# tfzhou/ContrastiveSeg

Measured on AMD Instinct MI355X. Metric: images/sec contrastive train step, HRNet-W48 1024x512 bs8, higher is better.
Workload: dtype fp32 in/out, f16x3 split MFMA (fp32 accumulate); 1 GPU; cfg2: BASELINE.json configs[1]: HRNet-W48 + contrast_ce_loss, synthetic Cityscapes 3x512x1024x19, tau=0.1, max_samples=1024, with_embed=True, SGD(0.01,0.9,5; model=hrnet_w48_contrast, loss=contrast_ce_loss, global_batch=8, per_gpu_batch=8, arithmetic=f16x3 on the matrix cores for the 3x3 / 1x1 convolutions, rest fp32, parallelism=dp1, step_graph=eager (auto: per-GPU batch above 1, the GPU is the limit)

## Files before the change

### contrastiveseg_amd/_hip.py

```python
import ctypes
import os

import torch

_PKG = os.path.dirname(os.path.abspath(__file__))
LIB_PATH = os.path.join(_PKG, "libcseg_hip.so")

_c_int = ctypes.c_int
_c_float = ctypes.c_float
_ptr = ctypes.c_void_p


class ContrastDesc(ctypes.Structure):
    _fields_ = [("mode", _c_int), ("N", _c_int), ("M", _c_int), ("D", _c_int),
                ("anchors", _ptr), ("a_lab", _ptr), ("contrast", _ptr), ("c_lab", _ptr),
                ("segment_queue", _ptr), ("pixel_queue", _ptr),
                ("bank_classes", _c_int), ("bank_size", _c_int),
                ("temperature", _c_float), ("base_temperature", _c_float)]


class ConvGroupMember(ctypes.Structure):
    _fields_ = [("x", _ptr), ("wp", _ptr), ("bias", _ptr), ("addend", _ptr), ("y", _ptr), ("stats", _ptr), ("amax_x", _ptr),
                ("amax_w", _ptr), ("B", _c_int), ("Cin", _c_int), ("Cout", _c_int), ("H", _c_int), ("W", _c_int),
                ("reserved", _c_int * 3)]


class BnGroupMember(ctypes.Structure):
    _fields_ = [("x", _ptr), ("residual", _ptr), ("y", _ptr), ("stats", _ptr), ("mean_invstd", _ptr), ("weight", _ptr), ("bias", _ptr),
                ("running_mean", _ptr), ("running_var", _ptr), ("num_batches_tracked", _ptr), ("amax_out", _ptr), ("dy", _ptr),
                ("out", _ptr), ("g_masked", _ptr), ("d_weight", _ptr), ("d_bias", _ptr), ("dx", _ptr), ("ws", _ptr),
                ("B", _c_int), ("C", _c_int), ("HW", _c_int), ("T", ctypes.c_long), ("eps", _c_float), ("momentum", _c_float)]


class WrwGroupMember(ctypes.Structure):
    _fields_ = [("x", _ptr), ("dy", _ptr), ("amax_x", _ptr), ("amax_dy", _ptr), ("ws", _ptr), ("dw", _ptr), ("B", _c_int), ("Cin", _c_int),
                ("Cout", _c_int), ("H", _c_int), ("W", _c_int), ("reserved", _c_int * 3)]


GROUP_MAX = 8
GROUP_SCHED_INTS = 320
NT_GROUP = 0x203


SIGNATURES = {
    "cseg_abi_version": (_c_int, []),
    "cseg_last_error": (ctypes.c_char_p, []),
    "cseg_classify_partition": (_c_int, [_ptr, _ptr, _ptr] + [_c_int] * 7 + [_ptr] * 7 + [_ptr]),
    "cseg_classify_partition_prezeroed": (_c_int, [_ptr, _ptr, _ptr] + [_c_int] * 7 + [_ptr] * 7 + [_ptr]),
    "cseg_gather_anchors": (_c_int, [_ptr, _c_int, _c_int, _c_int, _ptr, _ptr, _c_int, _ptr, _ptr, _ptr]),
    "cseg_scatter_anchor_grad": (_c_int, [_ptr, _c_int, _ptr, _c_int, _c_int, _c_int, _c_float, _ptr, _ptr]),
    "cseg_contrast_ws_bytes": (ctypes.c_size_t, [_c_int, _c_int]),
    "cseg_contrast_fwd": (_c_int, [ctypes.POINTER(ContrastDesc), _ptr, _ptr, _ptr, _ptr, _ptr]),
    "cseg_contrast_fused_ws_bytes": (ctypes.c_size_t, [_c_int, _c_int]),
    "cseg_contrast_fused_counter_offset": (ctypes.c_size_t, [_c_int, _c_int]),
    "cseg_contrast_fwd_fused": (_c_int, [ctypes.POINTER(ContrastDesc), _ptr, _ptr, _ptr, _ptr, _ptr, _ptr]),
    "cseg_contrast_bwd_parts": (_c_int, [_c_int, _c_int, _c_int]),
    "cseg_contrast_bwd": (_c_int, [ctypes.POINTER(ContrastDesc), _ptr, _ptr, _ptr, _ptr, _ptr]),
    "cseg_sampling_ws_ints": (ctypes.c_size_t, [_c_int] * 3),
    "cseg_sample_anchors": (_c_int, [_ptr, _ptr, _ptr] + [_c_int] * 5 + [_ptr] * 7 + [_ptr]),
    "cseg_mt_draw": (_c_int, [_ptr, _ptr, _ptr, _c_int, _ptr]),
    "cseg_gather_anchors_dn": (_c_int, [_ptr, _c_int, _c_int, _c_int, _ptr, _ptr, _ptr, _c_int, _ptr, _ptr, _ptr]),
    "cseg_contrast_fwd_dn": (_c_int, [_ptr, _ptr, _ptr, _c_int, _c_int, _c_float, _c_float, _ptr, _ptr, _ptr, _ptr, _ptr]),
    "cseg_contrast_bwd_parts_cap": (_c_int, [_c_int, _c_int]),
    "cseg_contrast_bwd_dn": (_c_int, [_ptr, _ptr, _ptr, _c_int, _c_int, _c_float, _ptr, _ptr, _ptr, _ptr, _ptr]),
    "cseg_scatter_anchor_grad_dn": (_c_int, [_ptr, _ptr, _ptr, _c_int, _c_int, _c_int, _c_int, _c_float, _ptr, _ptr]),
    "cseg_upcat_fwd": (_c_int, [_ptr, _ptr, _ptr, _ptr, _c_int, _c_int, _ptr, _ptr]),
    "cseg_upcat_fwd_amax": (_c_int, [_ptr, _ptr, _ptr, _ptr, _c_int, _c_int, _ptr, _ptr, _ptr]),
    "cseg_upcat_bwd": (_c_int, [_ptr, _ptr, _ptr, _ptr, _c_int, _c_int, _ptr, _ptr]),
    "cseg_fuse_sum_fwd": (_c_int, [_ptr, _c_int, _ptr, _ptr, _ptr, _c_int] + [_c_int] * 5 + [_ptr, _ptr]),
    "cseg_affine_channels": (_c_int, [_ptr, _ptr, _ptr, _c_int, _c_int, ctypes.c_long, _ptr, _ptr, _ptr]),
    "cseg_fuse_sum_fwd_amax": (_c_int, [_ptr, _c_int, _ptr, _ptr, _ptr, _c_int] + [_c_int] * 5 + [_ptr, _ptr, _ptr]),
    "cseg_fuse_sum_bwd": (_c_int, [_ptr, _ptr, _ptr, _ptr, _c_int] + [_c_int] * 4 + [_ptr, _ptr, _ptr]),
    "cseg_upsample_ce_blocks": (_c_int, [_c_int, _c_int, _c_int]),
    "cseg_upsample_ce_fwd": (_c_int, [_ptr, _ptr, _ptr, _c_int] + [_c_int] * 6 + [_ptr, _ptr, _ptr, _ptr, _ptr]),
    "cseg_upsample_ce_bwd": (_c_int, [_ptr, _ptr, _ptr, _c_int] + [_c_int] * 6 + [_ptr, _ptr, _ptr, _ptr, _ptr]),
    "cseg_queue_count": (_c_int, [_ptr, _c_int, _c_int, _c_int, _c_int, _c_int, _ptr, _ptr]),
    "cseg_queue_class_sums": (_c_int, [_ptr, _ptr] + [_c_int] * 7 + [_ptr, _ptr]),
    "cseg_queue_write_segments": (_c_int, [_ptr, _ptr, _ptr, _ptr, _ptr, _c_int, _c_int, _c_int, _ptr, _c_int, _ptr]),
    "cseg_queue_write_pixels": (_c_int, [_ptr, _c_int, _c_int, _c_int, _ptr, _ptr, _ptr, _ptr, _c_int, _ptr, _c_int,
                                         _ptr]),
    "cseg_conv3x3_packed_floats": (ctypes.c_size_t, [_c_int, _c_int]),
    "cseg_conv3x3_pack_weights": (_c_int, [_ptr, _c_int, _c_int, _c_int, _ptr, _ptr]),
    "cseg_conv3x3_fwd": (_c_int, [_ptr, _ptr, _c_int, _c_int, _c_int, _c_int, _c_int, _ptr, _ptr]),
    "cseg_conv3x3_wrw_ws_floats": (ctypes.c_size_t, [_c_int] * 5),
    "cseg_conv3x3_wrw": (_c_int, [_ptr, _ptr, _c_int, _c_int, _c_int, _c_int, _c_int, _ptr, _ptr, _ptr]),
    "cseg_conv3x3_sb_packed_bytes": (ctypes.c_size_t, [_c_int, _c_int]),
    "cseg_conv3x3_sb_pack_weights": (_c_int, [_ptr, _c_int, _c_int, _c_int, _ptr, _ptr]),
    "cseg_conv3x3_sb_fwd": (_c_int, [_ptr, _ptr, _ptr, _c_int, _c_int, _c_int, _c_int, _c_int, _ptr, _ptr]),
    "cseg_conv3x3_sb_pack_weights_nt": (_c_int, [_ptr, _c_int, _c_int, _c_int, _c_int, _ptr, _ptr]),
    "cseg_conv3x3_sb_fwd_nt": (_c_int, [_ptr, _ptr, _ptr, _c_int, _c_int, _c_int, _c_int, _c_int, _c_int, _ptr, _ptr]),
    "cseg_conv3x3_sb_wrw_ws_floats": (ctypes.c_size_t, [_c_int] * 5),
    "cseg_conv3x3_sb_wrw": (_c_int, [_ptr, _ptr, _c_int, _c_int, _c_int, _c_int, _c_int, _ptr, _ptr, _ptr]),
    "cseg_conv1x1_sb_packed_bytes": (ctypes.c_size_t, [_c_int, _c_int]),
    "cseg_conv1x1_sb_pack_weights": (_c_int, [_ptr, _c_int, _c_int, _c_int, _ptr, _ptr]),
    "cseg_conv1x1_sb_fwd": (_c_int, [_ptr, _ptr, _ptr, _c_int, _c_int, _c_int, _c_int, _ptr, _ptr]),
    "cseg_conv1x1_sb_wrw_ws_floats": (ctypes.c_size_t, [_c_int] * 4),
    "cseg_conv1x1_sb_wrw": (_c_int, [_ptr, _ptr, _c_int, _c_int, _c_int, _c_int, _ptr, _ptr, _ptr]),
    "cseg_amax_f32": (_c_int, [_ptr, ctypes.c_long, _ptr, _ptr]),
    "cseg_conv3x3_split_packed_bytes": (ctypes.c_size_t, [_c_int, _c_int, _c_int]),
    "cseg_conv3x3_split_pack": (_c_int, [_ptr, _c_int, _c_int, _c_int, _c_int, _c_int, _ptr, _ptr, _ptr]),
    "cseg_conv3x3_split_fwd": (_c_int, [_ptr, _ptr, _ptr] + [_c_int] * 7 + [_ptr, _ptr, _ptr, _ptr]),
    "cseg_conv3x3_split_wrw": (_c_int, [_ptr, _ptr] + [_c_int] * 6 + [_ptr, _ptr, _ptr, _ptr, _ptr]),
    "cseg_conv3x3_split_fwd_add": (_c_int, [_ptr, _ptr, _ptr, _ptr] + [_c_int] * 7 + [_ptr, _ptr, _ptr, _ptr]),
    "cseg_conv3x3_split_group_fwd": (_c_int, [_ptr, _c_int, _c_int, _ptr, _ptr]),
    "cseg_conv3x3_split_group_wrw": (_c_int, [_ptr, _c_int, _c_int, _ptr]),
    "cseg_bn_group_tiles_finalize": (_c_int, [_ptr, _c_int, _ptr]),
    "cseg_bn_group_apply": (_c_int, [_ptr, _c_int, _c_int, _ptr]),
    "cseg_bn_group_bwd": (_c_int, [_ptr, _c_int, _c_int, _c_int, _ptr]),
    "cseg_bn_group_tiles_moments": (_c_int, [_ptr, _c_int, _ptr, _ptr]),
    "cseg_bn_group_finalize": (_c_int, [_ptr, _c_int, _ptr, _ptr]),
    "cseg_bn_group_bwd_reduce": (_c_int, [_ptr, _c_int, _c_int, _ptr, _ptr]),
    "cseg_bn_group_bwd_apply": (_c_int, [_ptr, _c_int, _c_int, _ptr, _ptr]),
    "cseg_conv3x3_split_dil_fwd": (_c_int, [_ptr, _ptr, _ptr, _ptr] + [_c_int] * 7 + [_ptr, _ptr, _ptr, _ptr, _ptr]),
    "cseg_conv3x3_split_dilany_plan": (_c_int, [_c_int, _c_int, ctypes.POINTER(_c_int), ctypes.POINTER(ctypes.c_long)]),
    "cseg_conv3x3_split_dilany_packed_bytes": (ctypes.c_size_t, [_c_int] * 2),
    "cseg_conv3x3_split_dilany_pack": (_c_int, [_ptr, _c_int, _c_int, _c_int, _ptr, _ptr, _ptr]),
    "cseg_conv3x3_split_dilany_fwd": (_c_int, [_ptr, _ptr, _ptr, _ptr] + [_c_int] * 6 + [_ptr, _ptr, _ptr, _ptr, _ptr]),
    "cseg_conv3x3_split_dilany_wrw_ws_floats": (ctypes.c_size_t, [_c_int] * 6),
    "cseg_conv3x3_split_dilany_wrw": (_c_int, [_ptr, _ptr] + [_c_int] * 6 + [_ptr, _ptr, _ptr, _ptr, _ptr]),
    "cseg_conv3x3_s2_split_packed_bytes": (ctypes.c_size_t, [_c_int] * 2),
    "cseg_conv3x3_s2_split_plan": (_c_int, [_c_int] * 4 + [_ptr, _ptr]),
    "cseg_conv3x3_s2_split_pack": (_c_int, [_ptr] + [_c_int] * 4 + [_ptr, _ptr, _ptr]),
    "cseg_conv3x3_s2_split_fwd": (_c_int, [_ptr, _ptr] + [_c_int] * 6 + [_ptr, _ptr, _ptr, _ptr]),
    "cseg_conv3x3_s2_split_bwd": (_c_int, [_ptr, _ptr] + [_c_int] * 6 + [_ptr, _ptr, _ptr, _ptr]),
    "cseg_conv3x3_s2_rgb_fwd": (_c_int, [_ptr, _ptr] + [_c_int] * 4 + [_ptr, _ptr]),
    "cseg_conv3x3_s2_rgb_wrw_ws_floats": (ctypes.c_size_t, [_c_int] * 4),
    "cseg_conv3x3_s2_rgb_wrw": (_c_int, [_ptr, _ptr] + [_c_int] * 4 + [_ptr, _ptr, _ptr]),
    "cseg_cls1x1_fwd": (_c_int, [_ptr, _ptr, _ptr] + [_c_int] * 4 + [ctypes.c_long, _ptr, _ptr]),
    "cseg_cls1x1_bwd": (_c_int, [_ptr, _ptr] + [_c_int] * 4 + [ctypes.c_long, _ptr, _ptr]),
    "cseg_cls1x1_wrw_ws_floats": (ctypes.c_size_t, [_c_int, _c_int, _c_int, ctypes.c_long]),
    "cseg_cls1x1_wrw": (_c_int, [_ptr, _ptr] + [_c_int] * 4 + [ctypes.c_long, _ptr, _ptr, _ptr]),
    "cseg_cls1x1_wide_fwd": (_c_int, [_ptr, _ptr, _ptr] + [_c_int] * 4 + [ctypes.c_long, _ptr, _ptr]),
    "cseg_cls1x1_wide_bwd": (_c_int, [_ptr, _ptr] + [_c_int] * 4 + [ctypes.c_long, _ptr, _ptr]),
    "cseg_cls1x1_wide_wrw_ws_floats": (ctypes.c_size_t, [_c_int, _c_int, _c_int, ctypes.c_long]),
    "cseg_cls1x1_wide_wrw": (_c_int, [_ptr, _ptr] + [_c_int] * 4 + [ctypes.c_long, _ptr, _ptr, _ptr]),
    "cseg_ocr_gather_ws_floats": (ctypes.c_size_t, [_c_int] * 4 + [ctypes.c_long]),
    "cseg_ocr_gather_fwd": (_c_int, [_ptr, _ptr, _c_float] + [_c_int] * 4 + [ctypes.c_long, _ptr, _ptr, _ptr, _ptr]),
    "cseg_ocr_gather_bwd": (_c_int, [_ptr, _ptr, _ptr, _ptr, _c_float] + [_c_int] * 4 + [ctypes.c_long, _ptr, _ptr, _ptr]),
    "cseg_ocr_attn_fwd": (_c_int, [_ptr, _ptr, _ptr, _c_float] + [_c_int] * 4 + [ctypes.c_long, _ptr, _ptr, _ptr]),
    "cseg_ocr_attn_bwd_ws_floats": (ctypes.c_size_t, [_c_int] * 4 + [ctypes.c_long]),
    "cseg_ocr_attn_bwd": (_c_int, [_ptr] * 5 + [_c_float] + [_c_int] * 4 + [ctypes.c_long] + [_ptr] * 5),
    "cseg_conv3x3_s2_wrw_ws_floats": (ctypes.c_size_t, [_c_int] * 5),
    "cseg_conv3x3_s2_split_wrw": (_c_int, [_ptr, _ptr] + [_c_int] * 6 + [_ptr, _ptr, _ptr, _ptr, _ptr]),
    "cseg_conv1x1_split_packed_bytes": (ctypes.c_size_t, [_c_int, _c_int, _c_int]),
    "cseg_conv1x1_split_pack": (_c_int, [_ptr, _c_int, _c_int, _c_int, _c_int, _ptr, _ptr, _ptr]),
    "cseg_conv1x1_split_fwd": (_c_int, [_ptr, _ptr, _ptr] + [_c_int] * 5 + [_ptr, _ptr, _ptr, _ptr]),
    "cseg_conv1x1_split_fwd_add": (_c_int, [_ptr, _ptr, _ptr, _ptr] + [_c_int] * 5 + [_ptr, _ptr, _ptr, _ptr]),
    "cseg_conv1x1_split_wrw": (_c_int, [_ptr, _ptr] + [_c_int] * 5 + [_ptr, _ptr, _ptr, _ptr, _ptr]),
    "cseg_conv3x3_split_plan": (_c_int, [_c_int, _c_int, _c_int, _ptr, _ptr, _ptr]),
    "cseg_conv1x1_split_plan": (_c_int, [_c_int, _c_int, _ptr, _ptr]),
    "cseg_conv1x1_split_plan_arith": (_c_int, [_c_int, _c_int, _c_int, ctypes.POINTER(_c_int), ctypes.POINTER(ctypes.c_long)]),
    "cseg_amax_batch": (_c_int, [_ptr, _c_int, _c_int, _ptr]),
    "cseg_split_pack_batch": (_c_int, [_ptr, _c_int, _c_int, _c_int, _ptr]),
    "cseg_augment_batch": (_c_int, [_ptr, _ptr, _ptr, _ptr] + [_c_int] * 5 + [_c_float, _ptr, _ptr, _ptr, _ptr, _ptr]),
    "cseg_ms_fuse_argmax": (_c_int, [_c_int, ctypes.POINTER(_ptr), ctypes.POINTER(_ptr), ctypes.POINTER(_c_int), ctypes.POINTER(_c_int),
                                     ctypes.POINTER(_c_float)] + [_c_int] * 4 + [_ptr, _ptr, _ptr]),
    "cseg_confusion_update": (_c_int, [_ptr, _ptr, ctypes.c_long, _c_int, _c_int, _ptr, _ptr]),
    "cseg_rmi_pool_blocks": (_c_int, [_c_int] * 4),
    "cseg_rmi_pool_fwd": (_c_int, [_ptr, _ptr] + [_c_int] * 10 + [_ptr] * 5),
    "cseg_rmi_cov": (_c_int, [_ptr, _ptr] + [_c_int] * 4 + [_ptr, _ptr, _ptr]),
    "cseg_rmi_solve": (_c_int, [_ptr, _c_int, _ptr, _ptr, _ptr]),
    "cseg_rmi_finish": (_c_int, [_ptr, _c_int, _ptr, _c_int, _c_int, _c_float, _c_int, _c_float, _ptr, _ptr, _ptr]),
    "cseg_rmi_bwd": (_c_int, [_ptr] * 9 + [_c_int] * 6 + [_c_float, _c_int, _c_float, _ptr, _ptr, _ptr]),
    "cseg_lovasz_tiles": (_c_int, [ctypes.c_long]),
    "cseg_lovasz_errors": (_c_int, [_ptr, _ptr] + [_c_int] * 9 + [_ptr] * 6),
    "cseg_lovasz_pack": (_c_int, [_ptr, _ptr, _ptr, _c_int, _c_int, _ptr, _ptr]),
    "cseg_lovasz_order": (_c_int, [_ptr] * 5 + [_c_int, _c_int, _ptr]),
    "cseg_lovasz_grad": (_c_int, [_ptr, _ptr, _c_int, _c_int] + [_ptr] * 6),
    "cseg_lovasz_finish": (_c_int, [_ptr, _ptr, _c_int, _c_int] + [_ptr] * 4),
    "cseg_lovasz_bwd": (_c_int, [_ptr] * 5 + [_c_int] * 6 + [_ptr] * 3),
    "cseg_conv_stat_segments":(ctypes.c_size_t, [_c_int] * 4),
    "cseg_conv3x3_split_fwd_st": (_c_int, [_ptr, _ptr, _ptr] + [_c_int] * 7 + [_ptr, _ptr, _ptr, _ptr, _ptr]),
    "cseg_conv1x1_split_fwd_st": (_c_int, [_ptr, _ptr, _ptr] + [_c_int] * 5 + [_ptr, _ptr, _ptr, _ptr, _ptr]),
    "cseg_conv3x3_s2_split_fwd_st": (_c_int, [_ptr, _ptr] + [_c_int] * 6 + [_ptr, _ptr, _ptr, _ptr, _ptr]),
    "cseg_bn_tiles_finalize": (_c_int, [_ptr, _c_int, ctypes.c_long, _c_float, _c_float, _ptr, _ptr, _ptr, _ptr, _ptr]),
    "cseg_bn_tiles_moments": (_c_int, [_ptr, _c_int, ctypes.c_long, _ptr, _ptr]),
    "cseg_bn_ws_floats": (ctypes.c_size_t, [_c_int, _c_int, _c_int]),
    "cseg_bn_stats": (_c_int, [_ptr, _c_int, _c_int, _c_int, _ptr, _ptr, _ptr]),
    "cseg_bn_finalize": (_c_int, [_ptr, _c_int, ctypes.c_double, _c_float, _c_float, _ptr, _ptr, _ptr, _ptr, _ptr]),
    "cseg_bn_stats_finalize": (_c_int, [_ptr, _c_int, _c_int, _c_int, _ptr, _c_float, _c_float, _ptr, _ptr, _ptr, _ptr,
                                        _ptr]),
    "cseg_bn_fwd": (_c_int, [_ptr] * 4 + [_c_int] * 4 + [_ptr, _c_float, _c_float] + [_ptr] * 5 + [_ptr]),
    "cseg_bn_bwd": (_c_int, [_ptr] * 6 + [_c_int] * 5 + [_ptr] * 5 + [_ptr]),
    "cseg_bn_fwd_amax": (_c_int, [_ptr] * 4 + [_c_int] * 4 + [_ptr, _c_float, _c_float] + [_ptr] * 5 + [_ptr, _ptr]),
    "cseg_bn_bwd_amax": (_c_int, [_ptr] * 6 + [_c_int] * 5 + [_ptr] * 5 + [_ptr, _ptr]),
    "cseg_bn_apply_amax": (_c_int, [_ptr, _ptr, _ptr, _ptr, _ptr, _c_int, _c_int, _c_int, _c_int, _ptr, _ptr, _ptr]),
    "cseg_bn_bwd_apply_amax": (_c_int, [_ptr] * 6 + [ctypes.c_double, _c_int, _c_int, _c_int, _c_int, _ptr, _ptr, _ptr]),
    "cseg_bn_apply": (_c_int, [_ptr, _ptr, _ptr, _ptr, _ptr, _c_int, _c_int, _c_int, _c_int, _ptr, _ptr]),
# ... 56 lines not shown
```

### contrastiveseg_amd/csrc/conv1x1_sb_wrw.hip

```cpp
#include "cseg_split.h"

namespace {

constexpr int CO_T = 144, CI_T = 128, STG = 32;
constexpr int PITCH = 48;
__host__ __device__ constexpr int dy_elems(int np) { return np * CO_T * PITCH; }
__host__ __device__ constexpr int x_elems(int np) { return np * CI_T * PITCH; }
constexpr int CH_ALL = CO_T + CI_T;

constexpr int LD_ITEMS = CH_ALL * 8;
constexpr int LD_U = (LD_ITEMS + 255) / 256;

template <class AR, bool RAGGED = false>
__global__ __launch_bounds__(512, 1) void conv1x1_sb_wrw_kernel(const float* __restrict__ x, const float* __restrict__ dy,
                                                                int B, int Cin, int Cout, int plane_i, int n_split,
                                                                const unsigned* __restrict__ amax_x,
                                                                const unsigned* __restrict__ amax_dy,
                                                                float* __restrict__ partial) {
    extern __shared__ __attribute__((aligned(16))) unsigned short smem_q[];
    constexpr int NP = AR::NP;
    constexpr int DY_ELEMS = dy_elems(NP), X_ELEMS = x_elems(NP);
    typedef typename AR::frag_t frag_t;
    unsigned short* ds = smem_q;
    unsigned short* xs = smem_q + 2 * DY_ELEMS;
    const unsigned ex = AR::SCALED ? split_amax_exp(amax_x) : 141u, ed = AR::SCALED ? split_amax_exp(amax_dy) : 141u;
    const float xscale = split_scale_of(ex), dscale = split_scale_of(ed);
    const int tid = threadIdx.x, wave = __builtin_amdgcn_readfirstlane(tid >> 6), lane = tid & 63;
    const bool loader = wave >= 4;
    const int lt = tid - 256;
    const int g = lane >> 4, n = lane & 15;
    int blk = blockIdx.x;
    const int split = blk % n_split; blk /= n_split;
    const int n_cib = (Cin + CI_T - 1) / CI_T;
    const int cib = blk % n_cib;
    const int cob = blk / n_cib;
    const size_t plane = (size_t)plane_i;
    const int stages_per_img = RAGGED ? (plane_i + STG - 1) / STG : plane_i / STG;
    const long n_units = (long)B * stages_per_img;
    const long u_lo = n_units * split / n_split, u_hi = n_units * (split + 1) / n_split;

    if (loader) {
        unsigned off[LD_U];
        int lds_off[LD_U];
        int room[4] = {0, 0, 0, 0};
        int pc[LD_U];
        bool ok[LD_U], is_dy[LD_U];
#pragma unroll
        for (int u = 0; u < LD_U; ++u) {
            const int item = lt + 256 * u, itc = min(item, LD_ITEMS - 1);
            const int r = itc >> 3, c = itc & 7;
            is_dy[u] = 256 * u + 64 * (wave - 4) < CO_T * 8;
            const int ch = is_dy[u] ? min(cob * CO_T + r, Cout - 1) : min(cib * CI_T + r - CO_T, Cin - 1);
            off[u] = (unsigned)(ch * plane_i + 4 * c) * (unsigned)sizeof(float);
            ok[u] = item < LD_ITEMS && (is_dy[u] ? cob * CO_T + r < Cout : cib * CI_T + r - CO_T < Cin);
            lds_off[u] = is_dy[u] ? r * PITCH + 4 * c : (r - CO_T) * PITCH + 4 * c;
            pc[u] = 4 * c;
        }
        int img = (int)(u_lo / stages_per_img), stage = (int)(u_lo % stages_per_img);
        long next_unit = u_lo;
        auto load = [&](float4 (&v)[LD_U], int& room_of_set) __attribute__((always_inline)) {
            const float* dyp = dy + ((size_t)img * Cout * plane + (size_t)stage * STG);
            const float* xp = x + ((size_t)img * Cin * plane + (size_t)stage * STG);
#pragma unroll
            for (int u = 0; u < LD_U; ++u) {
                if (!RAGGED) {
                    v[u] = cseg_load_f4(is_dy[u] ? dyp : xp, off[u]);
                } else {
                    const int left = plane_i - stage * STG - pc[u];
                    const char* base = reinterpret_cast<const char*>(is_dy[u] ? dyp : xp) + off[u];
                    float e[4];
#pragma unroll
                    for (int k = 0; k < 4; ++k) e[k] = *reinterpret_cast<const float*>(base + (long)min(k, left - 1) * 4);
                    v[u] = make_float4(e[0], e[1], e[2], e[3]);
                }
            }
            room_of_set = plane_i - stage * STG;
            if (++next_unit < u_hi) {
                if (++stage == stages_per_img) { stage = 0; ++img; }
            }
        };
        auto put = [&](int buf, const float4 (&v)[LD_U], int room_of_set) __attribute__((always_inline)) {
#pragma unroll
            for (int u = 0; u < LD_U; ++u) {
                if (ok[u] || lt + 256 * u < LD_ITEMS) {
                    float4 t = ok[u] ? v[u] : make_float4(0.f, 0.f, 0.f, 0.f);
                    if (RAGGED) {
                        const int nv = room_of_set - pc[u];
                        t.x = nv > 0 ? t.x : 0.f; t.y = nv > 1 ? t.y : 0.f;
                        t.z = nv > 2 ? t.z : 0.f; t.w = nv > 3 ? t.w : 0.f;
                    }
                    uint2 cells[NP];
                    split_cells4<AR>(t, is_dy[u] ? dscale : xscale, cells);
                    unsigned short* base = is_dy[u] ? ds + buf * DY_ELEMS + lds_off[u] : xs + buf * X_ELEMS + lds_off[u];
                    const int pstride = is_dy[u] ? CO_T * PITCH : CI_T * PITCH;
#pragma unroll
                    for (int q = 0; q < NP; ++q) *reinterpret_cast<uint2*>(base + q * pstride) = cells[q];
                }
            }
        };
        constexpr int PF = 4;
        float4 v[PF][LD_U];
        if (u_lo < u_hi) {
            load(v[0], room[0]);
            put(0, v[0], room[0]);
#pragma unroll
            for (int s = 1; s < PF; ++s) load(v[s], room[s]);
            load(v[0], room[0]);
        }
        __syncthreads();
        long unit = u_lo;
#pragma unroll 1
        for (; unit + PF < u_hi; unit += PF) {
#pragma unroll
            for (int j = 0; j < PF; ++j) {
                put((j + 1) & 1, v[(j + 1) & 3], room[(j + 1) & 3]);
                load(v[(j + 1) & 3], room[(j + 1) & 3]);
                __syncthreads();
            }
        }
#pragma unroll
        for (int j = 0; j < PF; ++j) {
            if (unit + j < u_hi) {
                if (unit + j + 1 < u_hi) put((j + 1) & 1, v[(j + 1) & 3], room[(j + 1) & 3]);
                __syncthreads();
            }
        }
    } else {
        const int mh = wave & 1, nh = wave >> 1;
        const int cot0 = mh ? 5 : 0, cit0 = nh * 4;
        f32x4 acc[5][4];
#pragma unroll
        for (int a = 0; a < 5; ++a)
#pragma unroll
            for (int c = 0; c < 4; ++c) acc[a][c] = (f32x4){0.f, 0.f, 0.f, 0.f};
        __syncthreads();
        auto stage_mfmas = [&](int buf) __attribute__((always_inline)) {
            frag_t bf[4][NP];
#pragma unroll
            for (int c = 0; c < 4; ++c)
#pragma unroll
                for (int p = 0; p < NP; ++p)
                    bf[c][p] = __builtin_bit_cast(frag_t, *reinterpret_cast<const uint4*>(
                        xs + buf * X_ELEMS + (p * CI_T + (cit0 + c) * 16 + n) * PITCH + 8 * g));
#pragma unroll
            for (int a = 0; a < 5; ++a) {
                if (a == 4 && mh) break;
                frag_t af[NP];
#pragma unroll
                for (int p = 0; p < NP; ++p)
                    af[p] = __builtin_bit_cast(frag_t, *reinterpret_cast<const uint4*>(
                        ds + buf * DY_ELEMS + (p * CO_T + (cot0 + a) * 16 + n) * PITCH + 8 * g));
#pragma unroll
                for (int t = 0; t < AR::NTERMS; ++t)
#pragma unroll
                    for (int c = 0; c < 4; ++c) acc[a][c] = AR::mfma(af[AR::ta(t)], bf[c][AR::tb(t)], acc[a][c]);
            }
        };
#pragma unroll 1
        for (long unit = u_lo; unit < u_hi; unit += 2) {
#pragma unroll
            for (int j = 0; j < 2; ++j) {
                if (unit + j < u_hi) {
                    stage_mfmas(j);
                    __syncthreads();
                }
            }
        }
        const float unscale = split_unscale_of(ex) * split_unscale_of(ed);
#pragma unroll
        for (int a = 0; a < 5; ++a) {
            if (a == 4 && mh) break;
#pragma unroll
            for (int c = 0; c < 4; ++c) {
                const int ci = cib * CI_T + (cit0 + c) * 16 + n;
                const int co = cob * CO_T + (cot0 + a) * 16 + 4 * g;
                if (ci < Cin) {
#pragma unroll
                    for (int r = 0; r < 4; ++r)
                        if (co + r < Cout) partial[((size_t)split * Cout + co + r) * Cin + ci] = acc[a][c][r] * unscale;
                }
            }
        }
    }
}

__global__ __launch_bounds__(256) void sb_wrw1_reduce_kernel(const float* __restrict__ partial, int n_split, int total,
                                                             float* __restrict__ dw) {
    __shared__ float red[4][64];
    const int lane = threadIdx.x & 63, wave = threadIdx.x >> 6;
    const int e = blockIdx.x * 64 + lane;
    float s0 = 0.f, s1 = 0.f, s2 = 0.f, s3 = 0.f;
    if (e < total) {
        int sp = wave;
        for (; sp + 12 < n_split; sp += 16) {
            s0 += partial[(size_t)sp * total + e];
            s1 += partial[(size_t)(sp + 4) * total + e];
            s2 += partial[(size_t)(sp + 8) * total + e];
            s3 += partial[(size_t)(sp + 12) * total + e];
        }
        for (; sp < n_split; sp += 4) s0 += partial[(size_t)sp * total + e];
    }
    red[wave][lane] = (s0 + s1) + (s2 + s3);
    __syncthreads();
    if (wave == 0 && e < total) dw[e] = (red[0][lane] + red[1][lane]) + (red[2][lane] + red[3][lane]);
}

int wrw1_splits(int B, int Cin, int Cout, int plane) {
    const long units = (long)B * ((plane + STG - 1) / STG);
    const int pairs = ((Cin + CI_T - 1) / CI_T) * ((Cout + CO_T - 1) / CO_T);
    const double stage_us = 0.75, split_us = 2.0 * Cin * Cout * sizeof(float) / 4.0e6;
    const long n_max = units < 256 ? units : 256;
    auto cost_of = [&](long n) {
        const long rounds = (n * pairs + 255) / 256;
        return rounds * ((double)((units + n - 1) / n) * stage_us + 5.0) + n * split_us;
    };
    double best = 1e30;
    for (long n = 1; n <= n_max; ++n) best = cost_of(n) < best ? cost_of(n) : best;
    for (long n = 1; n <= n_max; ++n)
        if (cost_of(n) <= 1.03 * best) return (int)n;
    return (int)n_max;
}

}

extern "C" size_t cseg_conv1x1_sb_wrw_ws_floats(int B, int Cin, int Cout, int HW) {
    if (B <= 0 || Cin <= 0 || Cout <= 0 || HW <= 0 || Cin % 16 || Cout % 16) return 0;
    return (size_t)wrw1_splits(B, Cin, Cout, HW) * Cin * Cout;
}

namespace {
template <class AR, bool RAGGED>
int launch_wrw1(const float* x, const float* dy, int B, int Cin, int Cout, int HW, int n_split, long blocks, const unsigned* amax_x,
                const unsigned* amax_dy, float* ws, hipStream_t stream) {
    const size_t lds = sizeof(unsigned short) * 2 * (dy_elems(AR::NP) + x_elems(AR::NP));
    static bool attr_set = false;
    if (!attr_set) {
        if (hipFuncSetAttribute((const void*)conv1x1_sb_wrw_kernel<AR, RAGGED>, hipFuncAttributeMaxDynamicSharedMemorySize, (int)lds) !=
            hipSuccess) {
            cseg_set_error("conv1x1_sb_wrw: cannot raise dynamic LDS to %zu bytes", lds);
            return 0;
        }
        attr_set = true;
    }
    hipLaunchKernelGGL((conv1x1_sb_wrw_kernel<AR, RAGGED>), dim3((unsigned)blocks), dim3(512), lds, stream, x, dy, B, Cin, Cout, HW, n_split,
                       amax_x, amax_dy, ws);
    CSEG_CHECK_LAUNCH("conv1x1_sb_wrw_kernel");
    return 1;
}

int wrw1_impl(const float* x, const float* dy, int B, int Cin, int Cout, int HW, int arith, const unsigned* amax_x,
              const unsigned* amax_dy, float* ws, float* dw, hipStream_t stream) {
    CSEG_REQUIRE(x && dy && ws && dw, "conv1x1_sb_wrw: null pointer");
    CSEG_REQUIRE(B > 0 && HW > 0 && Cin > 0 && Cout > 0 && Cin % 16 == 0 && Cout % 16 == 0,
                 "conv1x1_sb_wrw: unsupported shape B=%d Cin=%d Cout=%d HW=%d (needs channels %% 16)", B, Cin, Cout, HW);
    const bool ragged = HW % STG != 0;
    CSEG_REQUIRE(ragged || ((reinterpret_cast<uintptr_t>(x) & 15) == 0 && (reinterpret_cast<uintptr_t>(dy) & 15) == 0),
                 "conv1x1_sb_wrw: tensors must be 16-byte aligned");
    CSEG_REQUIRE(arith == CSEG_ARITH_BF16X6 || (arith == CSEG_ARITH_F16X3 && amax_x && amax_dy),
                 "conv1x1 split wrw: arithmetic %d needs max|x| and max|dy|", arith);
    CSEG_REQUIRE((long)Cin * HW * 4 < 2147483647L && (long)Cout * HW * 4 < 2147483647L,
                 "conv1x1_sb_wrw: one image of x / dy must stay below 2 GiB (32-bit offsets)");
    const int n_split = wrw1_splits(B, Cin, Cout, HW);
    const long blocks = (long)n_split * ((Cin + CI_T - 1) / CI_T) * ((Cout + CO_T - 1) / CO_T);
    CSEG_REQUIRE(blocks < 2147483647L && (long)Cin * Cout < 2147483647L, "conv1x1_sb_wrw: grid too large");
    int ok;
    if (arith == CSEG_ARITH_F16X3)
        ok = ragged ? launch_wrw1<SplitF16x3, true>(x, dy, B, Cin, Cout, HW, n_split, blocks, amax_x, amax_dy, ws, stream)
                    : launch_wrw1<SplitF16x3, false>(x, dy, B, Cin, Cout, HW, n_split, blocks, amax_x, amax_dy, ws, stream);
    else
        ok = ragged ? launch_wrw1<SplitBF16x6, true>(x, dy, B, Cin, Cout, HW, n_split, blocks, amax_x, amax_dy, ws, stream)
                    : launch_wrw1<SplitBF16x6, false>(x, dy, B, Cin, Cout, HW, n_split, blocks, amax_x, amax_dy, ws, stream);
    if (!ok) return 0;
    const int total = Cin * Cout;
    hipLaunchKernelGGL(sb_wrw1_reduce_kernel, dim3((total + 63) / 64), dim3(256), 0, stream, ws, n_split, total, dw);
    CSEG_CHECK_LAUNCH("sb_wrw1_reduce_kernel");
    return 1;
}
}

extern "C" int cseg_conv1x1_sb_wrw(const float* x, const float* dy, int B, int Cin, int Cout, int HW, float* ws, float* dw,
                                   cseg_stream_t stream_) {
    return wrw1_impl(x, dy, B, Cin, Cout, HW, CSEG_ARITH_BF16X6, nullptr, nullptr, ws, dw, (hipStream_t)stream_);
}

extern "C" int cseg_conv1x1_split_wrw(const float* x, const float* dy, int B, int Cin, int Cout, int HW, int arith,
                                      const unsigned* amax_x, const unsigned* amax_dy, float* ws, float* dw, cseg_stream_t stream_) {
    return wrw1_impl(x, dy, B, Cin, Cout, HW, arith, amax_x, amax_dy, ws, dw, (hipStream_t)stream_);
}
```

### contrastiveseg_amd/csrc/conv3x3_sb_wrw.hip

```cpp
#include "cseg_split.h"
#include <stdlib.h>

namespace {

constexpr int CO_B = 48, CI_B = 64, SEG = 64;
constexpr int XP = 40;
constexpr int DP = 72;
constexpr int XS_ELEMS = 2 * 3 * CI_B * 3 * XP;
constexpr int DS_ELEMS = 3 * CO_B * DP;
constexpr int ROWS_PER_UNIT = 8;

__device__ __forceinline__ int xs_idx(int s, int p, int ci, int slot, int i) { return (((s * 3 + p) * CI_B + ci) * 3 + slot) * XP + i; }
__device__ __forceinline__ int ds_idx(int p, int co, int i) { return (p * CO_B + co) * DP + i; }

__device__ __forceinline__ void split8w(const float (&v)[8], uint4& h, uint4& m, uint4& l) {
    uint4 c[3];
    split_cells8<SplitBF16x6>(v, 1.f, c);
    h = c[0]; m = c[1]; l = c[2];
}

__global__ __launch_bounds__(512, 1) void conv3x3_sb_wrw_kernel(const float* __restrict__ x, const float* __restrict__ dy,
                                                                int B, int Cin, int Cout, int H, int W, int n_split,
                                                                float* __restrict__ partial) {
    extern __shared__ __attribute__((aligned(16))) unsigned short smem_w[];
// ... 106 lines not shown
                bfr[1][p] = __builtin_bit_cast(bf16x8, s1);
                bfr[2][p] = __builtin_bit_cast(bf16x8, s2);
            }
#define SBW_TERM(P, Q)                                                                                          \
    _Pragma("unroll") for (int kx = 0; kx < 3; ++kx) _Pragma("unroll") for (int c = 0; c < 3; ++c)             \
        acc[ky * 3 + kx][c] = __builtin_amdgcn_mfma_f32_16x16x32_bf16(a[c][P], bfr[kx][Q], acc[ky * 3 + kx][c], 0, 0, 0);
            SBW_TERM(2, 0)
            SBW_TERM(0, 2)
            SBW_TERM(1, 1)
            SBW_TERM(1, 0)
            SBW_TERM(0, 1)
            SBW_TERM(0, 0)
#undef SBW_TERM
        }
    };

    for (int unit = split; unit < n_units; unit += n_split) {
        int t = unit;
        const int run = t % runs; t /= runs;
        const int seg = t % segs;
        const int b = t / segs;
        const int x0 = seg * SEG, ya = run * ROWS_PER_UNIT, yb = min(ya + ROWS_PER_UNIT, H);
#pragma unroll 1
        for (int r = ya - 1; r <= ya + 1; ++r) {
            x_issue(b, x0, r);
            x_store(x0, r);
        }
        d_issue(b, x0, ya);
        d_store(ya);
        __syncthreads();
#pragma unroll 1
        for (int row = ya; row < yb; ++row) {
            const bool more = row + 1 < yb;
            if (more) {
                x_issue(b, x0, row + 2);
                d_issue(b, x0, row + 1);
            }
            if (tile_ok) compute(row);
            __syncthreads();
            if (more) {
                x_store(x0, row + 2);
                d_store(row + 1);
            }
            __syncthreads();
        }
    }

    float* red = reinterpret_cast<float*>(smem_w);
    if (ksl == 1 && tile_ok) {
#pragma unroll
        for (int t = 0; t < 9; ++t)
#pragma unroll
            for (int c = 0; c < 3; ++c)
                *reinterpret_cast<f32x4*>(red + (((sl * 27) + t * 3 + c) * 64 + lane) * 4) = acc[t][c];
    }
    __syncthreads();
    if (ksl == 0 && tile_ok) {
        const int ci = cib * CI_B + sl * 16 + n;
#pragma unroll
        for (int t = 0; t < 9; ++t)
#pragma unroll
            for (int c = 0; c < 3; ++c) {
                const f32x4 o = *reinterpret_cast<const f32x4*>(red + (((sl * 27) + t * 3 + c) * 64 + lane) * 4);
                const f32x4 v = acc[t][c] + o;
                float* dst = partial + (((size_t)split * 9 + t) * Cout + cob * CO_B + c * 16 + 4 * g) * Cin + ci;
#pragma unroll
                for (int r = 0; r < 4; ++r) dst[(size_t)r * Cin] = v[r];
            }
    }
}

__host__ __device__ constexpr int x2_lead(int np) { return np == 2 ? 8 : 4; }
__host__ __device__ constexpr int x2_slot(int np, int segw) { return segw + 2 * x2_lead(np); }
__host__ __device__ constexpr int x2_ch(int np, int segw) { return np == 2 ? (segw == 64 ? 336 : 208) : 4 * (segw + 8) + 8; }
__host__ __device__ constexpr int d2_pitch(int np, int segw) { return np == 2 ? (segw == 64 ? 80 : 48) : segw + 8; }
__host__ __device__ constexpr int x2_elems(int np, int segw) { return np * CI_B * x2_ch(np, segw); }
__host__ __device__ constexpr int d2_elems(int np, int segw) { return 2 * np * CO_B * d2_pitch(np, segw); }

template <int NP, int SEGW>
__device__ __forceinline__ int x2_idx(int p, int ci, int slot, int i) { return (p * CI_B + ci) * x2_ch(NP, SEGW) + slot * x2_slot(NP, SEGW) + i; }
template <int NP, int SEGW>
__device__ __forceinline__ int d2_idx(int buf, int p, int co, int i) { return ((buf * NP + p) * CO_B + co) * d2_pitch(NP, SEGW) + i; }

template <class AR, int SEGW, int ABL = 0, bool RAGGED = false>
__device__ __forceinline__ void conv3x3_sb_wrw2_body(const float* __restrict__ x, const float* __restrict__ dy,
                                                     int B, int Cin, int Cout, int H, int W, int n_split, int rpu,
                                                     int SC, int SI, const unsigned* __restrict__ amax_x,
                                                     const unsigned* __restrict__ amax_dy,
                                                     float* __restrict__ partial, int bid, unsigned short* smem_w) {
    constexpr int NP = AR::NP;
    typedef typename AR::frag_t frag_t;
    unsigned short* xs = smem_w;
    unsigned short* ds = smem_w + x2_elems(NP, SEGW);
    constexpr int XCH = x2_slot(NP, SEGW) / 4, XU = (CI_B * XCH + 255) / 256;
    constexpr int DCH = SEGW / 4, DU = (CO_B * DCH + 255) / 256;
    const unsigned ex = AR::SCALED ? split_amax_exp(amax_x) : 141u, ed = AR::SCALED ? split_amax_exp(amax_dy) : 141u;
    const float xscale = split_scale_of(ex), dscale = split_scale_of(ed);
    const int tid = threadIdx.x, wave = __builtin_amdgcn_readfirstlane(tid >> 6), lane = tid & 63;
    const bool loader = wave >= 4;
    const int lt = tid - 256;
    const int g = lane >> 4, n = lane & 15;
    const int n_cib = (Cin + CI_B - 1) / CI_B;
    int split, cib, cob;
    {
        const int n_cob = (Cout + CO_B - 1) / CO_B;
        const int n_si = n_cib / SI, gsz = SC * SI, n_groups = n_split * (n_cob / SC) * n_si;
        const int xcd = bid & 7, l = bid >> 3;
        const int grp = (l / gsz) * 8 + xcd, j = l % gsz;
        if (grp >= n_groups) return;
        split = grp % n_split;
        const int st = grp / n_split;
        cib = (st % n_si) * SI + j % SI;
        cob = (st / n_si) * SC + j / SI;
    }
    const size_t plane = (size_t)H * W;
    const int segs = RAGGED ? (W + SEGW - 1) / SEGW : W / SEGW;
    const int runs = (H + rpu - 1) / rpu;
    const int n_units = B * segs * runs;
    const bool tile_ok = !loader && cib * CI_B + wave * 16 < Cin;

    int xi_lds[XU], xi_px[XU], xi_ch[XU];
    bool xi_ok[XU];
#pragma unroll
    for (int u = 0; u < XU; ++u) {
        const int item = lt + 256 * u, itc = min(max(item, 0), CI_B * XCH - 1);
        const int ci = itc / XCH, c = itc - ci * XCH;
        xi_lds[u] = x2_idx<NP, SEGW>(0, ci, 0, 4 * c);
        xi_px[u] = 4 * c - x2_lead(NP);
        xi_ch[u] = min(cib * CI_B + ci, Cin - 1);
        xi_ok[u] = loader && item < CI_B * XCH && cib * CI_B + ci < Cin;
    }
    int di_lds[DU], di_off[DU], di_c4[DU];
    bool di_ok[DU];
#pragma unroll
    for (int u = 0; u < DU; ++u) {
        const int item = lt + 256 * u, itc = min(max(item, 0), CO_B * DCH - 1);
        const int co = itc / DCH, c = itc - co * DCH;
        di_lds[u] = d2_idx<NP, SEGW>(0, 0, co, 4 * c);
        di_c4[u] = 4 * c;
        di_off[u] = min(cob * CO_B + co, Cout - 1) * (int)plane + 4 * c;
        di_ok[u] = loader && item < CO_B * DCH && cob * CO_B + co < Cout;
    }
    const float* x_img = x;
    const float* d_img = dy;
    unsigned xu_off[XU], du_off[DU];
    bool xu_ok[XU];
    int xu_px[XU], du_px[DU];
    auto unit_setup = [&](int b, int x0) {
        x_img = x + (size_t)b * Cin * plane;
        d_img = dy + (size_t)b * Cout * plane;
#pragma unroll
        for (int u = 0; u < XU; ++u) {
            const int px = x0 + xi_px[u];
            if (RAGGED) {
                xu_off[u] = (unsigned)(xi_ch[u] * (int)plane) * (unsigned)sizeof(float);
                xu_px[u] = px;
                xu_ok[u] = xi_ok[u];
            } else {
                xu_off[u] = (unsigned)(xi_ch[u] * (int)plane + min(max(px, 0), W - 4)) * (unsigned)sizeof(float);
                xu_ok[u] = xi_ok[u] && px >= 0 && px < W;
            }
        }
#pragma unroll
        for (int u = 0; u < DU; ++u) {
            if (RAGGED) {
                du_off[u] = (unsigned)(di_off[u] - di_c4[u]) * (unsigned)sizeof(float);
                du_px[u] = x0 + di_c4[u];
            } else {
                du_off[u] = (unsigned)(di_off[u] + x0) * (unsigned)sizeof(float);
            }
        }
    };
// ... 142 lines not shown
        }
    };

    auto unit_dims = [&](int unit, int& b, int& x0, int& ya, int& yb) {
        int t = unit;
        const int run = t % runs; t /= runs;
        const int seg = t % segs;
        b = t / segs;
        x0 = seg * SEGW; ya = run * rpu; yb = min(ya + rpu, H);
    };

    if (loader) {
        for (int unit = split; unit < n_units; unit += n_split) {
            int b, x0, ya, yb;
            unit_dims(unit, b, x0, ya, yb);
            unit_setup(b, x0);
            float4 xv[XU], dv[DU];
            {
                float4 x0v[XU], x1v[XU];
                x_load(ya - 1, x0v);
                x_load(ya, x1v);
                x_load(ya + 1, xv);
                d_load(ya, dv);
                x_put(ya - 1, 0, x0v);
                x_put(ya, 1, x1v);
                x_put(ya + 1, 2, xv);
                d_put(0, dv);
            }
            if (ya + 1 < yb) {
                x_load(ya + 2, xv);
                d_load(ya + 1, dv);
            }
            __syncthreads();
#pragma unroll 1
            for (int r0 = ya; r0 < yb; r0 += 4) {
#pragma unroll
                for (int j = 0; j < 4; ++j) {
                    const int row = r0 + j;
                    if (row < yb) {
                        if (row + 1 < yb) {
                            if (!(ABL & 8)) {
                                x_put(row + 2, (j + 3) & 3, xv);
                                d_put((j + 1) & 1, dv);
                            }
                            if (row + 2 < yb) {
                                x_load(row + 3, xv);
                                d_load(row + 2, dv);
                            }
                        }
                        __syncthreads();
                    }
                }
            }
        }
    } else {
        f32x4 acc[9][3];
#pragma unroll
        for (int t = 0; t < 9; ++t)
#pragma unroll
            for (int c = 0; c < 3; ++c) acc[t][c] = (f32x4){0.f, 0.f, 0.f, 0.f};
        for (int unit = split; unit < n_units; unit += n_split) {
            int b, x0, ya, yb;
            unit_dims(unit, b, x0, ya, yb);
            __syncthreads();
#pragma unroll 1
            for (int r0 = ya; r0 < yb; r0 += 4) {
#pragma unroll
                for (int j = 0; j < 4; ++j) {
                    if (r0 + j < yb) {
                        if (tile_ok) compute(j, j & 1, acc);
                        __syncthreads();
                    }
                }
            }
        }
        if (tile_ok) {
            const int ci = cib * CI_B + wave * 16 + n;
            const float unscale = split_unscale_of(ex) * split_unscale_of(ed);
#pragma unroll
            for (int t = 0; t < 9; ++t)
#pragma unroll
                for (int c = 0; c < 3; ++c) {
                    if (cob * CO_B + c * 16 >= Cout) continue;
                    float* dst = partial + (((size_t)split * 9 + t) * Cout + cob * CO_B + c * 16 + 4 * g) * Cin + ci;
#pragma unroll
                    for (int r = 0; r < 4; ++r) dst[(size_t)r * Cin] = acc[t][c][r] * unscale;
                }
        }
    }
}

template <class AR, int SEGW, int ABL = 0, bool RAGGED = false>
__global__ __launch_bounds__(512, 1) void conv3x3_sb_wrw2_kernel(const float* __restrict__ x, const float* __restrict__ dy,
                                                                 int B, int Cin, int Cout, int H, int W, int n_split, int rpu,
                                                                 int SC, int SI, const unsigned* __restrict__ amax_x,
                                                                 const unsigned* __restrict__ amax_dy,
                                                                 float* __restrict__ partial) {
    extern __shared__ __attribute__((aligned(16))) unsigned short smem_w2[];
    conv3x3_sb_wrw2_body<AR, SEGW, ABL, RAGGED>(x, dy, B, Cin, Cout, H, W, n_split, rpu, SC, SI, amax_x, amax_dy, partial, (int)blockIdx.x, smem_w2);
}

__device__ __forceinline__ void sb_wrw_reduce_body(const float* __restrict__ partial, int n_split, int Cout, int Cin,
                                                   float* __restrict__ dw, int bid) {
    __shared__ float red[4][64];
    const int lane = threadIdx.x & 63, wave = threadIdx.x >> 6;
    const int e = bid * 64 + lane;
    const int total = 9 * Cout * Cin;
    float s0 = 0.f, s1 = 0.f, s2 = 0.f, s3 = 0.f;
    if (e < total) {
        int sp = wave;
        for (; sp + 12 < n_split; sp += 16) {
            s0 += partial[(size_t)sp * total + e];
            s1 += partial[(size_t)(sp + 4) * total + e];
            s2 += partial[(size_t)(sp + 8) * total + e];
            s3 += partial[(size_t)(sp + 12) * total + e];
        }
        for (; sp < n_split; sp += 4) s0 += partial[(size_t)sp * total + e];
    }
    red[wave][lane] = (s0 + s1) + (s2 + s3);
    __syncthreads();
    if (wave == 0 && e < total) {
        const float v = (red[0][lane] + red[1][lane]) + (red[2][lane] + red[3][lane]);
        const int ci = e % Cin, rest = e / Cin;
        const int co = rest % Cout, tap = rest / Cout;
        dw[((size_t)co * Cin + ci) * 9 + tap] = v;
    }
}
__global__ __launch_bounds__(256) void sb_wrw_reduce_kernel(const float* __restrict__ partial, int n_split, int Cout, int Cin,
                                                            float* __restrict__ dw) {
    sb_wrw_reduce_body(partial, n_split, Cout, Cin, dw, (int)blockIdx.x);
}

int sb_wrw_version() {
    const char* e = getenv("CSEG_CONV3X3_SB_WRW_V");
    return e && atoi(e) == 1 ? 1 : 2;
}

int wrw2_seg(int W) { return W % 64 == 0 ? 64 : (W % 32 == 0 ? 32 : (W > 48 ? 64 : 32)); }
bool wrw2_ragged(int W) { return W % wrw2_seg(W) != 0; }
int wrw2_rpu(int H) { return H >= 32 ? 16 : 8; }

void sb_wrw_group(int n_cob, int n_cib, int& SC, int& SI);

int sb_wrw_splits(int B, int Cin, int Cout, int H, int W, int arith) {
    const bool v2 = arith == CSEG_ARITH_F16X3 || sb_wrw_version() == 2;
    const int rpu = v2 ? wrw2_rpu(H) : ROWS_PER_UNIT;
    const int seg = v2 ? wrw2_seg(W) : SEG;
    const int units = B * ((W + seg - 1) / seg) * ((H + rpu - 1) / rpu);
    const int n_cib = (Cin + CI_B - 1) / CI_B, n_cob = (Cout + CO_B - 1) / CO_B;
    const int pairs = n_cib * n_cob;
    if (!v2) {
        int n = (768 + pairs - 1) / pairs;
        if (n > 256) n = 256;
        if (n > units) n = units;
        return n < 1 ? 1 : n;
    }
    int SC, SI;
    sb_wrw_group(n_cob, n_cib, SC, SI);
    const int gsz = SC * SI, groups_per_split = (n_cob / SC) * (n_cib / SI);
    const double unit_us = rpu * (seg / 32) * 1.15;
    const double split_us = 2.0 * 9.0 * Cin * Cout * sizeof(float) / 4.0e6;
    const char* force = getenv("CSEG_SB_WRW_SPLITS");
    if (force && atoi(force) > 0) return atoi(force) < units ? atoi(force) : units;
    auto cost_of = [&](int n) {
        const long per_xcd = ((long)n * groups_per_split + 7) / 8 * gsz;
        const long rounds = (per_xcd + 31) / 32;
        return rounds * ((double)((units + n - 1) / n) * unit_us + 5.0) + n * split_us;
    };
    const int n_max = units < 256 ? units : 256;
    double best_cost = 1e30;
    for (int n = 1; n <= n_max; ++n) best_cost = cost_of(n) < best_cost ? cost_of(n) : best_cost;
    for (int n = 1; n <= n_max; ++n)
        if (cost_of(n) <= 1.03 * best_cost) return n;
    return n_max;
}

}

extern "C" size_t cseg_conv3x3_sb_wrw_ws_floats(int B, int Cin, int Cout, int H, int W) {
    if (B <= 0 || Cin <= 0 || Cout <= 0 || H <= 0 || W <= 0 || Cin % 16 || Cout % 16) return 0;
    if (Cout % CO_B) return (size_t)sb_wrw_splits(B, Cin, Cout, H, W, CSEG_ARITH_F16X3) * 9 * Cin * Cout;
    if (W % 32) return (size_t)sb_wrw_splits(B, Cin, Cout, H, W, CSEG_ARITH_F16X3) * 9 * Cin * Cout;
    if (W % SEG && sb_wrw_version() != 2) return (size_t)sb_wrw_splits(B, Cin, Cout, H, W, CSEG_ARITH_F16X3) * 9 * Cin * Cout;
    const int a = sb_wrw_splits(B, Cin, Cout, H, W, CSEG_ARITH_BF16X6), b = sb_wrw_splits(B, Cin, Cout, H, W, CSEG_ARITH_F16X3);
    return (size_t)(a > b ? a : b) * 9 * Cin * Cout;
}

namespace {

void sb_wrw_group(int n_cob, int n_cib, int& SC, int& SI) {
    SC = SI = 1;
    double best = CO_B + CI_B;
    for (int sc = 1; sc <= n_cob; ++sc) {
        if (n_cob % sc) continue;
        for (int si = 1; si <= n_cib && sc * si <= 32; ++si) {
            if (n_cib % si) continue;
            const double per_block = (double)(sc * CO_B + si * CI_B) / (sc * si);
            if (per_block < best - 1e-9) { best = per_block; SC = sc; SI = si; }
        }
    }
}

template <class AR, int SEGW, int ABL = 0, bool RAGGED = false>
int launch_wrw2(const float* x, const float* dy, int B, int Cin, int Cout, int H, int W, int n_split, const unsigned* amax_x,
                const unsigned* amax_dy, float* ws, hipStream_t stream) {
    const size_t lds2 = sizeof(unsigned short) * (x2_elems(AR::NP, SEGW) + d2_elems(AR::NP, SEGW));
    static bool attr2_set = false;
    if (!attr2_set) {
        if (hipFuncSetAttribute((const void*)(conv3x3_sb_wrw2_kernel<AR, SEGW, ABL, RAGGED>), hipFuncAttributeMaxDynamicSharedMemorySize, (int)lds2) !=
            hipSuccess) {
            cseg_set_error("conv3x3_sb_wrw: cannot raise dynamic LDS to %zu bytes", lds2);
            return 0;
        }
        attr2_set = true;
    }
    const int n_cob = (Cout + CO_B - 1) / CO_B, n_cib = (Cin + CI_B - 1) / CI_B;
    int SC, SI;
    sb_wrw_group(n_cob, n_cib, SC, SI);
    const long n_groups = (long)n_split * (n_cob / SC) * (n_cib / SI);
    const long blocks = ((n_groups + 7) / 8) * 8 * SC * SI;
    CSEG_REQUIRE(blocks < 2147483647L, "conv3x3_sb_wrw: grid too large");
    hipLaunchKernelGGL((conv3x3_sb_wrw2_kernel<AR, SEGW, ABL, RAGGED>), dim3((unsigned)blocks), dim3(512), lds2, stream, x, dy, B, Cin, Cout, H, W,
                       n_split, wrw2_rpu(H), SC, SI, amax_x, amax_dy, ws);
    CSEG_CHECK_LAUNCH("conv3x3_sb_wrw2_kernel");
    return 1;
}

int wrw_impl(const float* x, const float* dy, int B, int Cin, int Cout, int H, int W, int arith, const unsigned* amax_x,
             const unsigned* amax_dy, float* ws, float* dw, hipStream_t stream) {
    CSEG_REQUIRE(x && dy && ws && dw, "conv3x3_sb_wrw: null pointer");
    const bool v2 = arith == CSEG_ARITH_F16X3 || sb_wrw_version() == 2;
    const bool ragged = v2 && arith == CSEG_ARITH_F16X3 && wrw2_ragged(W);
    CSEG_REQUIRE(B > 0 && H > 0 && W > 0 && Cin > 0 && Cout > 0 && Cin % 16 == 0 && Cout % 16 == 0 &&
                     (Cout % CO_B == 0 || (v2 && arith == CSEG_ARITH_F16X3)) && (ragged || W % (v2 ? 32 : SEG) == 0),
                 "conv3x3_sb_wrw: unsupported shape B=%d Cin=%d Cout=%d %dx%d (needs Cin %% 16, Cout %% 48 -- f16x3: Cout %% 16; bf16x6: W %% 32; version 1: W %% 64)",
                 B, Cin, Cout, H, W);
    CSEG_REQUIRE(arith == CSEG_ARITH_BF16X6 || (arith == CSEG_ARITH_F16X3 && amax_x && amax_dy),
                 "conv3x3 split wrw: arithmetic %d needs max|x| and max|dy|", arith);
    const int n_split = sb_wrw_splits(B, Cin, Cout, H, W, arith);
    const long blocks = (long)n_split * ((Cin + CI_B - 1) / CI_B) * ((Cout + CO_B - 1) / CO_B);
    CSEG_REQUIRE(blocks < 2147483647L && (long)9 * Cin * Cout < 2147483647L, "conv3x3_sb_wrw: grid too large");
    if (v2) {
        CSEG_REQUIRE(ragged || ((reinterpret_cast<uintptr_t>(x) & 15) == 0 && (reinterpret_cast<uintptr_t>(dy) & 15) == 0),
                     "conv3x3_sb_wrw: tensors must be 16-byte aligned");
        CSEG_REQUIRE((long)Cin * H * W * 4 < 2147483647L && (long)Cout * H * W * 4 < 2147483647L,
                     "conv3x3_sb_wrw: one image of x / dy must stay below 2 GiB (32-bit offsets)");
        const bool wide = wrw2_seg(W) == 64;
        const int ok = ragged
                           ? (wide ? launch_wrw2<SplitF16x3, 64, 0, true>(x, dy, B, Cin, Cout, H, W, n_split, amax_x, amax_dy, ws, stream)
                                   : launch_wrw2<SplitF16x3, 32, 0, true>(x, dy, B, Cin, Cout, H, W, n_split, amax_x, amax_dy, ws, stream))
                       : arith == CSEG_ARITH_F16X3
                           ? (wide ? launch_wrw2<SplitF16x3, 64>(x, dy, B, Cin, Cout, H, W, n_split, amax_x, amax_dy, ws, stream)
                                   : launch_wrw2<SplitF16x3, 32>(x, dy, B, Cin, Cout, H, W, n_split, amax_x, amax_dy, ws, stream))
                           : (wide ? launch_wrw2<SplitBF16x6, 64>(x, dy, B, Cin, Cout, H, W, n_split, amax_x, amax_dy, ws, stream)
                                   : launch_wrw2<SplitBF16x6, 32>(x, dy, B, Cin, Cout, H, W, n_split, amax_x, amax_dy, ws, stream));
        if (!ok) return 0;
    } else {
        const size_t lds = sizeof(unsigned short) * (XS_ELEMS + DS_ELEMS);
        static bool attr_set = false;
        if (!attr_set) {
            if (hipFuncSetAttribute((const void*)conv3x3_sb_wrw_kernel, hipFuncAttributeMaxDynamicSharedMemorySize,
                                    (int)lds) != hipSuccess) {
                cseg_set_error("conv3x3_sb_wrw: cannot raise dynamic LDS to %zu bytes", lds);
                return 0;
            }
            attr_set = true;
        }
        hipLaunchKernelGGL(conv3x3_sb_wrw_kernel, dim3((unsigned)blocks), dim3(512), lds, stream, x, dy, B, Cin, Cout, H, W,
                           n_split, ws);
        CSEG_CHECK_LAUNCH("conv3x3_sb_wrw_kernel");
    }
    const int total = 9 * Cin * Cout;
    hipLaunchKernelGGL(sb_wrw_reduce_kernel, dim3((total + 63) / 64), dim3(256), 0, stream, ws, n_split, Cout, Cin, dw);
    CSEG_CHECK_LAUNCH("sb_wrw_reduce_kernel");
    return 1;
}


struct WrwGM {
    const float* x; const float* dy; const unsigned* amax_x; const unsigned* amax_dy; float* ws; float* dw;
    int B, Cin, Cout, H, W, n_split, rpu, SC, SI, kind, block0, rblock0;
};
struct WrwGArgs { WrwGM m[CSEG_GROUP_MAX]; int n; };

template <int SEGW>
__global__ __launch_bounds__(512, 1) void conv3x3_wrw2_group_kernel(const WrwGArgs a) {
    extern __shared__ __attribute__((aligned(16))) unsigned short smem_wg[];
    int mi = 0;
    for (int i = 1; i < a.n; ++i) mi = (int)blockIdx.x >= a.m[i].block0 ? i : mi;
    const WrwGM& M = a.m[mi];
    conv3x3_sb_wrw2_body<SplitF16x3, SEGW, 0, false>(M.x, M.dy, M.B, M.Cin, M.Cout, M.H, M.W, M.n_split, M.rpu, M.SC, M.SI, M.amax_x, M.amax_dy, M.ws,
                                                     (int)blockIdx.x - M.block0, smem_wg);
}
__global__ __launch_bounds__(256) void sb_wrw_reduce_group_kernel(const WrwGArgs a) {
    int mi = 0;
    for (int i = 1; i < a.n; ++i) mi = (int)blockIdx.x >= a.m[i].rblock0 ? i : mi;
    const WrwGM& M = a.m[mi];
    sb_wrw_reduce_body(M.ws, M.n_split, M.Cout, M.Cin, M.dw, (int)blockIdx.x - M.rblock0);
}

template <int SEGW>
int launch_wrw2_group(const WrwGArgs& a, long blocks, hipStream_t stream) {
    const size_t lds = sizeof(unsigned short) * (x2_elems(2, SEGW) + d2_elems(2, SEGW));
    static bool attr_set = false;
    if (!attr_set) {
        if (hipFuncSetAttribute((const void*)conv3x3_wrw2_group_kernel<SEGW>, hipFuncAttributeMaxDynamicSharedMemorySize, (int)lds) != hipSuccess) {
            cseg_set_error("conv3x3 group wrw: cannot raise dynamic LDS to %zu bytes", lds);
            return 0;
        }
        attr_set = true;
    }
    hipLaunchKernelGGL(conv3x3_wrw2_group_kernel<SEGW>, dim3((unsigned)blocks), dim3(512), lds, stream, a);
    CSEG_CHECK_LAUNCH("conv3x3_wrw2_group_kernel");
    return 1;
}

int wrw_group_impl(const cseg_wrw_group_member* mem, int n, hipStream_t stream) {
    bool any_ragged = false;
    for (int i = 0; i < n; ++i) {
        const cseg_wrw_group_member& s = mem[i];
        CSEG_REQUIRE(s.x && s.dy && s.ws && s.dw && s.amax_x && s.amax_dy, "conv3x3 group wrw: member %d has a null pointer", i);
        CSEG_REQUIRE(s.B > 0 && s.H > 0 && s.W > 0 && s.Cin > 0 && s.Cout > 0 && s.Cin % 16 == 0 && s.Cout % CO_B == 0,
                     "conv3x3 group wrw: member %d: unsupported shape B=%d Cin=%d Cout=%d %dx%d (needs Cin %% 16, Cout %% 48)", i, s.B, s.Cin, s.Cout,
                     s.H, s.W);
        any_ragged = any_ragged || wrw2_ragged(s.W);
    }
    if (any_ragged) {
        for (int i = 0; i < n; ++i)
            if (!wrw_impl(mem[i].x, mem[i].dy, mem[i].B, mem[i].Cin, mem[i].Cout, mem[i].H, mem[i].W, CSEG_ARITH_F16X3, mem[i].amax_x, mem[i].amax_dy,
                          mem[i].ws, mem[i].dw, stream))
                return 0;
        return 1;
    }
    WrwGArgs all;
    long rblocks = 0;
    for (int i = 0; i < n; ++i) {
        const cseg_wrw_group_member& s = mem[i];
        CSEG_REQUIRE((reinterpret_cast<uintptr_t>(s.x) & 15) == 0 && (reinterpret_cast<uintptr_t>(s.dy) & 15) == 0,
                     "conv3x3 group wrw: member %d: tensors must be 16-byte aligned", i);
        CSEG_REQUIRE((long)s.Cin * s.H * s.W * 4 < 2147483647L && (long)s.Cout * s.H * s.W * 4 < 2147483647L && (long)9 * s.Cin * s.Cout < 2147483647L,
                     "conv3x3 group wrw: member %d: one image of x / dy must stay below 2 GiB (32-bit offsets)", i);
        WrwGM& m = all.m[i];
        m.x = s.x; m.dy = s.dy; m.amax_x = s.amax_x; m.amax_dy = s.amax_dy; m.ws = s.ws; m.dw = s.dw;
        m.B = s.B; m.Cin = s.Cin; m.Cout = s.Cout; m.H = s.H; m.W = s.W;
        m.n_split = sb_wrw_splits(s.B, s.Cin, s.Cout, s.H, s.W, CSEG_ARITH_F16X3);
        m.rpu = wrw2_rpu(s.H);
        const int n_cob = s.Cout / CO_B, n_cib = (s.Cin + CI_B - 1) / CI_B;
        sb_wrw_group(n_cob, n_cib, m.SC, m.SI);
        m.kind = wrw2_seg(s.W) == 64 ? 0 : 1;
        m.block0 = 0;
        m.rblock0 = (int)rblocks;
        rblocks += (9L * s.Cin * s.Cout + 63) / 64;
        CSEG_REQUIRE(rblocks < 2147483647L, "conv3x3 group wrw: grid too large");
    }
    for (int i = n; i < CSEG_GROUP_MAX; ++i) all.m[i] = all.m[0];
    all.n = n;
    for (int kind = 0; kind < 2; ++kind) {
        WrwGArgs a;
        long blocks = 0;
        int k = 0;
        for (int i = 0; i < n; ++i) {
            if (all.m[i].kind != kind) continue;
            a.m[k] = all.m[i];
            const WrwGM& m = a.m[k];
            const long n_groups = (long)m.n_split * ((m.Cout / CO_B) / m.SC) * (((m.Cin + CI_B - 1) / CI_B) / m.SI);
            a.m[k].block0 = (int)blocks;
            blocks += ((n_groups + 7) / 8) * 8 * m.SC * m.SI;
            CSEG_REQUIRE(blocks < 2147483647L, "conv3x3 group wrw: grid too large");
            ++k;
        }
        if (k == 0) continue;
        for (int i = k; i < CSEG_GROUP_MAX; ++i) a.m[i] = a.m[0];
        a.n = k;
        if (!(kind == 0 ? launch_wrw2_group<64>(a, blocks, stream) : launch_wrw2_group<32>(a, blocks, stream))) return 0;
    }
    hipLaunchKernelGGL(sb_wrw_reduce_group_kernel, dim3((unsigned)rblocks), dim3(256), 0, stream, all);
    CSEG_CHECK_LAUNCH("sb_wrw_reduce_group_kernel");
    return 1;
}

}

extern "C" int cseg_conv3x3_split_group_wrw(const cseg_wrw_group_member* mem, int n, int arith, cseg_stream_t stream_) {
    CSEG_REQUIRE(mem && n >= 1 && n <= CSEG_GROUP_MAX, "conv3x3 group wrw: needs 1 .. %d members", CSEG_GROUP_MAX);
    CSEG_REQUIRE(arith == CSEG_ARITH_F16X3, "conv3x3 group wrw: f16x3 arithmetic only (got %d)", arith);
    return wrw_group_impl(mem, n, (hipStream_t)stream_);
}

namespace {

constexpr int S2_SEG = 32;
constexpr int S2_PL = S2_SEG + 8;
constexpr int S2_ROWIMG = 2 * S2_PL;
constexpr int S2_XCH = 432;
constexpr int S2_DP = 48;
constexpr int S2_KCH = S2_SEG / 2 + 2;
constexpr int s2_x_elems(int np) { return np * CI_B * S2_XCH; }
constexpr int s2_d_elems(int np) { return 2 * np * CO_B * S2_DP; }

template <class AR>
__global__ __launch_bounds__(512, 1) void conv3x3_sb_wrw_s2_kernel(const float* __restrict__ x, const float* __restrict__ dy,
                                                                   int B, int Cin, int Cout, int Ho, int Wo, int n_split, int rpu,
                                                                   int SC, int SI, const unsigned* __restrict__ amax_x,
                                                                   const unsigned* __restrict__ amax_dy,
                                                                   float* __restrict__ partial) {
    extern __shared__ __attribute__((aligned(16))) unsigned short smem_w[];
    constexpr int NP = AR::NP;
    typedef typename AR::frag_t frag_t;
    unsigned short* xs = smem_w;
    unsigned short* ds = smem_w + s2_x_elems(NP);
    constexpr int XU = (CI_B * S2_KCH + 255) / 256;
    constexpr int DCH = S2_SEG / 4, DU = (CO_B * DCH + 255) / 256;
    const unsigned ex = split_amax_exp(amax_x), ed = split_amax_exp(amax_dy);
    const float xscale = split_scale_of(ex), dscale = split_scale_of(ed);
    const int tid = threadIdx.x, wave = __builtin_amdgcn_readfirstlane(tid >> 6), lane = tid & 63;
    const bool loader = wave >= 4;
    const int lt = tid - 256;
    const int g = lane >> 4, n = lane & 15;
    const int n_cib = (Cin + CI_B - 1) / CI_B;
    int split, cib, cob;
    {
        const int n_cob = (Cout + CO_B - 1) / CO_B;
        const int n_si = n_cib / SI, gsz = SC * SI, n_groups = n_split * (n_cob / SC) * n_si;
        const int xcd = blockIdx.x & 7, l = blockIdx.x >> 3;
        const int grp = (l / gsz) * 8 + xcd, j = l % gsz;
        if (grp >= n_groups) return;
        split = grp % n_split;
        const int st = grp / n_split;
        cib = (st % n_si) * SI + j % SI;
        cob = (st / n_si) * SC + j / SI;
    }
    const int H = 2 * Ho, W = 2 * Wo;
    const size_t plane = (size_t)H * W, oplane = (size_t)Ho * Wo;
    const int segs = Wo / S2_SEG;
    const int runs = (Ho + rpu - 1) / rpu;
    const int n_units = B * segs * runs;
    const bool tile_ok = !loader && cib * CI_B + wave * 16 < Cin;

    auto x_at = [&](int p, int ci, int slot, int pl, int i) { return xs + (p * CI_B + ci) * S2_XCH + slot * S2_ROWIMG + pl * S2_PL + i; };
    auto d_at = [&](int buf, int p, int co, int i) { return ds + ((buf * NP + p) * CO_B + co) * S2_DP + i; };

    int xi_lds[XU], xi_px[XU], xi_ch[XU];
    bool xi_ok[XU];
#pragma unroll
    for (int u = 0; u < XU; ++u) {
        const int item = lt + 256 * u, itc = min(max(item, 0), CI_B * S2_KCH - 1);
        const int ci = itc / S2_KCH, k = itc - ci * S2_KCH + 2;
        xi_lds[u] = (int)(x_at(0, ci, 0, 0, 2 * k) - xs);
        xi_px[u] = 4 * k - 16;
        xi_ch[u] = min(cib * CI_B + ci, Cin - 1);
        xi_ok[u] = loader && item < CI_B * S2_KCH && cib * CI_B + ci < Cin;
    }
    int di_lds[DU], di_off[DU];
    bool di_ok[DU];
#pragma unroll
    for (int u = 0; u < DU; ++u) {
        const int item = lt + 256 * u, itc = min(max(item, 0), CO_B * DCH - 1);
        const int co = itc / DCH, c = itc - co * DCH;
        di_lds[u] = (int)(d_at(0, 0, co, 4 * c) - ds);
        di_off[u] = min(cob * CO_B + co, Cout - 1) * (int)oplane + 4 * c;
        di_ok[u] = loader && item < CO_B * DCH && cob * CO_B + co < Cout;
    }
    const float* x_img = x;
    const float* d_img = dy;
    unsigned xu_off[XU], du_off[DU];
    bool xu_ok[XU];
    auto unit_setup = [&](int b, int x0) {
        x_img = x + (size_t)b * Cin * plane;
        d_img = dy + (size_t)b * Cout * oplane;
#pragma unroll
        for (int u = 0; u < XU; ++u) {
            const int px = 2 * x0 + xi_px[u];
            xu_off[u] = (unsigned)(xi_ch[u] * (int)plane + min(max(px, 0), W - 4)) * (unsigned)sizeof(float);
            xu_ok[u] = xi_ok[u] && px >= 0 && px < W;
        }
#pragma unroll
        for (int u = 0; u < DU; ++u) du_off[u] = (unsigned)(di_off[u] + x0) * (unsigned)sizeof(float);
    };
    auto x_load = [&](int row, float4 (&v)[XU]) __attribute__((always_inline)) {
        const float* rowp = x_img + (size_t)min(max(row, 0), H - 1) * W;
#pragma unroll
        for (int u = 0; u < XU; ++u) v[u] = cseg_load_f4(rowp, xu_off[u]);
    };
    auto x_put = [&](int row, int slot, const float4 (&v)[XU]) __attribute__((always_inline)) {
        const bool row_ok = row >= 0 && row < H;
#pragma unroll
        for (int u = 0; u < XU; ++u) {
            if (xi_ok[u]) {
// ... 67 lines not shown
#pragma unroll
                for (int kx = 0; kx < 3; ++kx)
#pragma unroll
                    for (int c = 0; c < 3; ++c)
                        acc[ky * 3 + kx][c] = AR::mfma(a[c][AR::ta(t)], bfr[kx][AR::tb(t)], acc[ky * 3 + kx][c]);
        }
    };

    auto unit_dims = [&](int unit, int& b, int& x0, int& ya, int& yb) {
        int t = unit;
        const int run = t % runs; t /= runs;
        const int seg = t % segs;
        b = t / segs;
        x0 = seg * S2_SEG; ya = run * rpu; yb = min(ya + rpu, Ho);
    };

    if (loader) {
        for (int unit = split; unit < n_units; unit += n_split) {
            int b, x0, ya, yb;
            unit_dims(unit, b, x0, ya, yb);
            unit_setup(b, x0);
            float4 ev[XU], ov[XU], dv[DU];
            {
                float4 o0v[XU];
                x_load(2 * ya - 1, o0v);
                x_load(2 * ya, ev);
                x_load(2 * ya + 1, ov);
                d_load(ya, dv);
                x_put(2 * ya - 1, 2, o0v);
                x_put(2 * ya, 0, ev);
                x_put(2 * ya + 1, 3, ov);
                d_put(0, dv);
            }
            if (ya + 1 < yb) {
                x_load(2 * ya + 2, ev);
                x_load(2 * ya + 3, ov);
                d_load(ya + 1, dv);
            }
            __syncthreads();
            int m3 = 0;
#pragma unroll 1
            for (int row = ya; row < yb; ++row) {
                const int k = row - ya;
                if (row + 1 < yb) {
                    x_put(2 * row + 2, (k + 1) & 1, ev);
                    x_put(2 * row + 3, 2 + (m3 == 0 ? 2 : m3 - 1), ov);
                    d_put((k + 1) & 1, dv);
                    if (row + 2 < yb) {
                        x_load(2 * row + 4, ev);
                        x_load(2 * row + 5, ov);
                        d_load(row + 2, dv);
                    }
                }
                __syncthreads();
                m3 = m3 == 2 ? 0 : m3 + 1;
            }
        }
    } else {
        f32x4 acc[9][3];
#pragma unroll
        for (int t = 0; t < 9; ++t)
#pragma unroll
            for (int c = 0; c < 3; ++c) acc[t][c] = (f32x4){0.f, 0.f, 0.f, 0.f};
        for (int unit = split; unit < n_units; unit += n_split) {
            int b, x0, ya, yb;
            unit_dims(unit, b, x0, ya, yb);
            __syncthreads();
            int m3 = 0;
#pragma unroll 1
            for (int row = ya; row < yb; ++row) {
                if (tile_ok) compute(row - ya, m3, acc);
                __syncthreads();
                m3 = m3 == 2 ? 0 : m3 + 1;
            }
        }
        if (tile_ok) {
            const int ci = cib * CI_B + wave * 16 + n;
            const float unscale = split_unscale_of(ex) * split_unscale_of(ed);
#pragma unroll
            for (int t = 0; t < 9; ++t)
#pragma unroll
                for (int c = 0; c < 3; ++c) {
                    if (cob * CO_B + c * 16 >= Cout) continue;
                    float* dst = partial + (((size_t)split * 9 + t) * Cout + cob * CO_B + c * 16 + 4 * g) * Cin + ci;
#pragma unroll
                    for (int r = 0; r < 4; ++r) dst[(size_t)r * Cin] = acc[t][c][r] * unscale;
                }
        }
    }
}

void s2_plan(int B, int Cin, int Cout, int Ho, int Wo, int& rpu, int& n_split) {
    const int pairs = ((Cin + CI_B - 1) / CI_B) * ((Cout + CO_B - 1) / CO_B);
    int want = (768 + pairs - 1) / pairs;
    if (want > 256) want = 256;
    rpu = 4;
    const char* force = getenv("CSEG_S2_WRW_RPU");
    const int forced = force ? atoi(force) : 0;
    for (int r = 16; r >= 4; r >>= 1) {
        if (forced > 0) { rpu = forced; break; }
        const long units = (long)B * (Wo / S2_SEG) * ((Ho + r - 1) / r);
        if (units * pairs >= 256 || r == 4) { rpu = r; break; }
    }
    const long units = (long)B * (Wo / S2_SEG) * ((Ho + rpu - 1) / rpu);
    n_split = (int)(want < units ? want : units);
    if (n_split < 1) n_split = 1;
}

bool s2_shape_ok(int B, int Cin, int Cout, int Ho, int Wo) {
    return B > 0 && Cin > 0 && Cout > 0 && Ho > 0 && Wo > 0 && Cin % 16 == 0 && Cout % 16 == 0 && Wo % S2_SEG == 0;
}

}

extern "C" size_t cseg_conv3x3_s2_wrw_ws_floats(int B, int Cin, int Cout, int Ho, int Wo) {
    if (!s2_shape_ok(B, Cin, Cout, Ho, Wo)) return 0;
    int rpu, n_split;
    s2_plan(B, Cin, Cout, Ho, Wo, rpu, n_split);
    return (size_t)n_split * 9 * Cin * Cout;
}

extern "C" int cseg_conv3x3_s2_split_wrw(const float* x, const float* dy, int B, int Cin, int Cout, int Ho, int Wo, int arith,
                                         const unsigned* amax_x, const unsigned* amax_dy, float* ws, float* dw,
                                         cseg_stream_t stream_) {
    hipStream_t stream = (hipStream_t)stream_;
    CSEG_REQUIRE(x && dy && ws && dw, "conv3x3_s2_wrw: null pointer");
    CSEG_REQUIRE(s2_shape_ok(B, Cin, Cout, Ho, Wo), "conv3x3_s2_wrw: unsupported shape B=%d Cin=%d Cout=%d out %dx%d (needs Cin %% 16, Cout %% 16, Wo %% 32)",
                 B, Cin, Cout, Ho, Wo);
    CSEG_REQUIRE(arith == CSEG_ARITH_F16X3 && amax_x && amax_dy, "conv3x3_s2_wrw: f16x3 only (needs max|x| and max|dy|)");
    CSEG_REQUIRE((reinterpret_cast<uintptr_t>(x) & 15) == 0 && (reinterpret_cast<uintptr_t>(dy) & 15) == 0,
                 "conv3x3_s2_wrw: tensors must be 16-byte aligned");
    CSEG_REQUIRE((long)9 * Cin * Cout < 2147483647L, "conv3x3_s2_wrw: too large");
    CSEG_REQUIRE((long)Cin * Ho * Wo * 16 < 2147483647L && (long)Cout * Ho * Wo * 4 < 2147483647L,
                 "conv3x3_s2_wrw: one image of x / dy must stay below 2 GiB (32-bit offsets)");
    int rpu, n_split;
    s2_plan(B, Cin, Cout, Ho, Wo, rpu, n_split);
    const size_t lds = sizeof(unsigned short) * (s2_x_elems(2) + s2_d_elems(2));
    static bool attr_set = false;
    if (!attr_set) {
        if (hipFuncSetAttribute((const void*)(conv3x3_sb_wrw_s2_kernel<SplitF16x3>), hipFuncAttributeMaxDynamicSharedMemorySize, (int)lds) !=
            hipSuccess) {
            cseg_set_error("conv3x3_s2_wrw: cannot raise dynamic LDS to %zu bytes", lds);
            return 0;
        }
        attr_set = true;
    }
    const int n_cob = (Cout + CO_B - 1) / CO_B, n_cib = (Cin + CI_B - 1) / CI_B;
    int SC, SI;
    sb_wrw_group(n_cob, n_cib, SC, SI);
    const long n_groups = (long)n_split * (n_cob / SC) * (n_cib / SI);
    const long blocks = ((n_groups + 7) / 8) * 8 * SC * SI;
    CSEG_REQUIRE(blocks < 2147483647L, "conv3x3_s2_wrw: grid too large");
    hipLaunchKernelGGL((conv3x3_sb_wrw_s2_kernel<SplitF16x3>), dim3((unsigned)blocks), dim3(512), lds, stream, x, dy, B, Cin, Cout, Ho, Wo,
                       n_split, rpu, SC, SI, amax_x, amax_dy, ws);
    CSEG_CHECK_LAUNCH("conv3x3_sb_wrw_s2_kernel");
    const int total = 9 * Cin * Cout;
    hipLaunchKernelGGL(sb_wrw_reduce_kernel, dim3((total + 63) / 64), dim3(256), 0, stream, ws, n_split, Cout, Cin, dw);
    CSEG_CHECK_LAUNCH("sb_wrw_reduce_kernel");
    return 1;
}

extern "C" int cseg_conv3x3_sb_wrw(const float* x, const float* dy, int B, int Cin, int Cout, int H, int W, float* ws,
                                   float* dw, cseg_stream_t stream_) {
    return wrw_impl(x, dy, B, Cin, Cout, H, W, CSEG_ARITH_BF16X6, nullptr, nullptr, ws, dw, (hipStream_t)stream_);
}

extern "C" int cseg_conv3x3_split_wrw(const float* x, const float* dy, int B, int Cin, int Cout, int H, int W, int arith,
                                      const unsigned* amax_x, const unsigned* amax_dy, float* ws, float* dw,
                                      cseg_stream_t stream_) {
    return wrw_impl(x, dy, B, Cin, Cout, H, W, arith, amax_x, amax_dy, ws, dw, (hipStream_t)stream_);
}
```

### contrastiveseg_amd/csrc/cseg_common.h

```cpp
#pragma once
#include <stdlib.h>
#include <hip/hip_runtime.h>
#include <stdint.h>
#include <stdio.h>
#include "cseg_hip.h"

#define CSEG_WAVE 64

#ifndef CSEG_WAVE_LOCKSTEP
#define CSEG_WAVE_LOCKSTEP()                                  \
    do {                                                      \
        __builtin_amdgcn_fence(__ATOMIC_RELEASE, "wavefront"); \
        __builtin_amdgcn_wave_barrier();                      \
    } while (0)
#endif

#ifndef CSEG_KEEP_DWORD
#define CSEG_KEEP_DWORD(v) asm volatile("" ::"v"(v))
#endif

__device__ __forceinline__ float4 cseg_load_f4(const void* uniform_base, unsigned byte_offset) {
    return *reinterpret_cast<const float4*>(static_cast<const char*>(uniform_base) + byte_offset);
}

__device__ __forceinline__ void cseg_release_agent() {
#if defined(__AMDGCN__)
    __builtin_amdgcn_fence(__ATOMIC_RELEASE, "agent");
    asm volatile("s_waitcnt vmcnt(0)" ::: "memory");
#else
    __atomic_thread_fence(__ATOMIC_SEQ_CST);
#endif
}
__device__ __forceinline__ void cseg_acquire_agent() {
#if defined(__AMDGCN__)
    __builtin_amdgcn_fence(__ATOMIC_ACQUIRE, "agent");
#else
    __atomic_thread_fence(__ATOMIC_SEQ_CST);
#endif
}
__device__ __forceinline__ int cseg_counter_add(int* p, int v) {
#if defined(__AMDGCN__)
    return __hip_atomic_fetch_add(p, v, __ATOMIC_RELAXED, __HIP_MEMORY_SCOPE_AGENT);
#else
    return __atomic_fetch_add(p, v, __ATOMIC_SEQ_CST);
#endif
}
__device__ __forceinline__ int cseg_counter_load(const int* p) {
#if defined(__AMDGCN__)
    return __hip_atomic_load(p, __ATOMIC_RELAXED, __HIP_MEMORY_SCOPE_AGENT);
#else
    return __atomic_load_n(p, __ATOMIC_SEQ_CST);
#endif
}
__device__ __forceinline__ void cseg_counter_store(int* p, int v) {
#if defined(__AMDGCN__)
    __hip_atomic_store(p, v, __ATOMIC_RELAXED, __HIP_MEMORY_SCOPE_AGENT);
#else
    __atomic_store_n(p, v, __ATOMIC_SEQ_CST);
#endif
}
#ifndef CSEG_SPIN_PAUSE
#if defined(__AMDGCN__)
#define CSEG_SPIN_PAUSE() __builtin_amdgcn_s_sleep(16)
#else
#define CSEG_SPIN_PAUSE() ((void)0)
#endif
#endif
#ifndef CSEG_GRID_RESIDENT_LAUNCH
#define CSEG_GRID_RESIDENT_LAUNCH() ((void)0)
#endif
__device__ __forceinline__ void cseg_wait_counter(const int* counter, int want) {
    for (long spins = 0; cseg_counter_load(counter) < want; ++spins) {
        CSEG_SPIN_PAUSE();
        if (spins > (1L << 25)) __builtin_trap();
    }
}

typedef float cseg_f32x4 __attribute__((ext_vector_type(4)));
__device__ __forceinline__ void cseg_store_row4(float* __restrict__ orow, const float* __restrict__ arow, long xx, long W, bool vec,
                                                cseg_f32x4 v) {
    if (vec && xx + 3 < W) {
        if (arow) {
            const float4 ad = *reinterpret_cast<const float4*>(arow + xx);
            v[0] += ad.x; v[1] += ad.y; v[2] += ad.z; v[3] += ad.w;
        }
        *reinterpret_cast<float4*>(orow + xx) = make_float4(v[0], v[1], v[2], v[3]);
    } else {
#pragma unroll
        for (int k = 0; k < 4; ++k)
            if (xx + k < W) orow[xx + k] = v[k] + (arow ? arow[xx + k] : 0.f);
    }
}

void cseg_set_error(const char* fmt, ...);

__device__ __forceinline__ int cseg_xcd_block(int b, int n, int on) { return (on && (n & 7) == 0) ? (b & 7) * (n >> 3) + (b >> 3) : b; }
static inline int cseg_xcd_remap() {
    const char* e = getenv("CSEG_XCD_REMAP");
    return e && atoi(e) == 0 ? 0 : 1;
}

#define CSEG_CHECK_LAUNCH(name)                                                     \
    do {                                                                            \
        hipError_t e__ = hipGetLastError();                                         \
        if (e__ != hipSuccess) {                                                    \
            cseg_set_error("%s: %s", name, hipGetErrorString(e__));                 \
            return 0;                                                               \
        }                                                                           \
    } while (0)

#define CSEG_REQUIRE(cond, ...)                                                     \
    do {                                                                            \
        if (!(cond)) {                                                              \
            cseg_set_error(__VA_ARGS__);                                            \
            return 0;                                                               \
        }                                                                           \
    } while (0)

__device__ __forceinline__ float wave_sum(float v) {
#pragma unroll
    for (int o = 32; o > 0; o >>= 1) v += __shfl_xor(v, o, 64);
    return v;
}
__device__ __forceinline__ float wave_max(float v) {
#pragma unroll
    for (int o = 32; o > 0; o >>= 1) v = fmaxf(v, __shfl_xor(v, o, 64));
    return v;
}
__device__ __forceinline__ int wave_sum_i(int v) {
#pragma unroll
    for (int o = 32; o > 0; o >>= 1) v += __shfl_xor(v, o, 64);
    return v;
}
__device__ __forceinline__ int wave_incl_scan_i(int v, int lane) {
#pragma unroll
    for (int o = 1; o < 64; o <<= 1) {
        int n = __shfl_up(v, o, 64);
        if (lane >= o) v += n;
    }
    return v;
}

// ... 4 lines not shown
```

### contrastiveseg_amd/kernels.py

```python
import ctypes

import os

import torch
from torch.autograd import Function
from torch.autograd.function import once_differentiable

from . import _hip

I32, I16, I64, F32 = torch.int32, torch.int16, torch.int64, torch.float32


def _p(t, dtype, what):
    return _hip.dev(t, dtype, what)


def _null():
    return ctypes.c_void_p(None)


def _on_device(t):
    return t.is_cuda


# ... 1354 lines not shown
    return (kh, kw) == (3, 3) and ok(ci) and ok(co) and x.shape[1] == ci


NT_SB8 = 0x109
CONV3X3_SB8 = os.environ.get("CSEG_CONV3X3_SB8", "1") == "1"


def conv3x3_sb_head_nt(c_out, x=None):
    if not (CONV3X3_SB8 and SPLIT_ARITH == "f16x3" and c_out % 144 == 0):
        return 0
    if x is not None and x.shape[0] * ((x.shape[2] + 7) // 8) * ((x.shape[3] + 63) // 64) * (c_out // 144) < 1024:
        return 0
    return NT_SB8


def conv3x3_sb_pick_nt(x, c_out):
    cands = [nt for nt in (9, 6, 3) if c_out % (16 * nt) == 0]
    spatial = x.shape[0] * ((x.shape[2] + 3) // 4) * ((x.shape[3] + 63) // 64)
    for nt in cands:
        if spatial * (c_out // (16 * nt)) >= 256:
            return nt
    return cands[-1]


def conv3x3_sb_pack(weight, transpose_flip=False, nt=0):
    return SPLIT_WEIGHTS.get(weight, "c3", transpose_flip, nt)


def conv3x3_sb_run(x, weight, transpose_flip=False, bias=None, nt=0, ax=None, addend=None, want_stats=False):
    co, ci = weight.shape[:2]
    conv_in, conv_out = (co, ci) if transpose_flip else (ci, co)
    B, _, H, W = x.shape
    arith = split_arith_id()
    wp, aw = conv3x3_sb_pack(weight, transpose_flip, nt)
    if arith and ax is None:
        ax = tensor_amax(x)
    y = torch.empty(B, conv_out, H, W, dtype=F32, device=x.device)
    if addend is not None:
        if tuple(addend.shape) != tuple(y.shape):
            raise RuntimeError("conv3x3_sb_run: addend %s does not have the output's shape %s" % (tuple(addend.shape), tuple(y.shape)))
        _hip.call("cseg_conv3x3_split_fwd_add", _pq(x, "x"), wp.data_ptr(), _opt(bias, F32, "bias"), _p(addend, F32, "addend"), B,
                  conv_in, conv_out, H, W, int(nt), arith, _pf(ax) if arith else _null(), _pf(aw) if arith else _null(), _pf(y),
                  _hip.stream_ptr())
        return y
    if want_stats and CONV_EPILOGUE_STATS:
        st = tile_stats_buffer(0, conv_out, B, H, W, x.device)
        _hip.call("cseg_conv3x3_split_fwd_st", _pq(x, "x"), wp.data_ptr(), _opt(bias, F32, "bias"), B, conv_in, conv_out, H, W,
                  int(nt), arith, _pf(ax) if arith else _null(), _pf(aw) if arith else _null(), _pf(y), _pf(st), _hip.stream_ptr())
        return tile_stats_attach(y, st)
    _hip.call("cseg_conv3x3_split_fwd", _pq(x, "x"), wp.data_ptr(), _opt(bias, F32, "bias"), B, conv_in, conv_out, H, W,
              int(nt), arith, _pf(ax) if arith else _null(), _pf(aw) if arith else _null(), _pf(y), _hip.stream_ptr())
    return y


CONV3X3_SB_MIN_TILES = int(os.environ.get("CSEG_SB_MIN_TILES", "1"))


def conv3x3_sb_tiles(x, c_out):
    if c_out in CONV3X3_SB_PICK_NT_CHANNELS:
        nt16 = 16 * conv3x3_sb_pick_nt(x, c_out)
    else:
        nt16 = 144 if c_out % 144 == 0 else 96 if c_out % 96 == 0 else 48 if c_out % 48 == 0 else 64
    return x.shape[0] * (c_out // nt16) * ((x.shape[2] + 3) // 4) * ((x.shape[3] + 63) // 64)


CONV3X3_SB_WRW = os.environ.get("CSEG_CONV3X3_SB_WRW", "1") == "1"
CONV3X3_SB_WRW_CHANNELS = tuple(int(c) for c in os.environ.get("CSEG_CONV3X3_SB_WRW_CHANNELS", "48,64,96,128,192,384,720").split(","))


CONV3X3_SB_WRW_PAIRS = ((256, 48),)


def conv3x3_sb_wrw_eligible(x, dy):
    return (_on_device(x) and x.dtype == F32 and dy.dtype == F32 and x.is_contiguous() and dy.is_contiguous()
            and x.shape[1] % 16 == 0 and (dy.shape[1] % 48 == 0 or (dy.shape[1] % 16 == 0 and SPLIT_ARITH == "f16x3"))
            and (x.shape[3] % 32 == 0 or SPLIT_ARITH == "f16x3"))


def conv3x3_sb_wrw_wanted(x, dy):
    same = x.shape[1] == dy.shape[1] and x.shape[1] in CONV3X3_SB_WRW_CHANNELS
    return CONV3X3_SB_WRW and (same or (x.shape[1], dy.shape[1]) in CONV3X3_SB_WRW_PAIRS) and conv3x3_sb_wrw_eligible(x, dy)


def conv3x3_sb_wrw(x, dy, ax=None, ady=None):
    B, ci, H, W = x.shape
    co = dy.shape[1]
    lib = _hip.lib()
    n = lib.cseg_conv3x3_sb_wrw_ws_floats(B, ci, co, H, W)
    if n == 0:
        raise RuntimeError("conv3x3_sb_wrw: unsupported shape %s x %s" % (tuple(x.shape), tuple(dy.shape)))
    arith = split_arith_id()
    if arith:
        ax = tensor_amax(x) if ax is None else ax
        ady = tensor_amax(dy) if ady is None else ady
    ws = torch.empty(n, dtype=F32, device=x.device)
    dw = torch.empty(co, ci, 3, 3, dtype=F32, device=x.device)
    _hip.call("cseg_conv3x3_split_wrw", _pq(x, "x"), _pq(dy, "dy"), B, ci, co, H, W, arith,
              _pf(ax) if arith else _null(), _pf(ady) if arith else _null(), _pf(ws), _pf(dw), _hip.stream_ptr())
    return dw


def mark_zero_channel_sum(dx):
    if dx is not None:
        dx._cseg_zero_chan_sum = dx._version
    return dx


BIAS_GRAD_SHORTCUT = os.environ.get("CSEG_BIAS_GRAD_SHORTCUT", "1") == "1"


def bias_grad(dy):
    if BIAS_GRAD_SHORTCUT and getattr(dy, "_cseg_zero_chan_sum", None) == dy._version:
        return torch.zeros(dy.shape[1], dtype=dy.dtype, device=dy.device)
    return dy.sum((0, 2, 3))


class Conv3x3SplitBF16(Function):

    @staticmethod
    def forward(ctx, x, weight, bias, want_stats=False):
        weight = weight.contiguous()
        ctx.save_for_backward(x, weight)
        ctx.has_bias = bias is not None
        ctx.pick = weight.shape[0] in CONV3X3_SB_PICK_NT_CHANNELS
        ctx.ax = amax_of(x) if split_arith_id() else None
        nt = conv3x3_sb_pick_nt(x, weight.shape[0]) if ctx.pick else conv3x3_sb_head_nt(weight.shape[0], x)
        return conv3x3_sb_run(x, weight, False, bias, nt, ax=ctx.ax, want_stats=want_stats)

    @staticmethod
    def backward(ctx, dy):
        x, weight = ctx.saved_tensors
        ady = amax_of(dy) if split_arith_id() else None
        dy = dy.contiguous()
        dx = None
        if ctx.needs_input_grad[0]:
            nt = conv3x3_sb_pick_nt(dy, weight.shape[1]) if ctx.pick else conv3x3_sb_head_nt(weight.shape[1], dy)
            dx = conv3x3_sb_run(dy, weight, True, None, nt, ax=ady)
        dw = db = None
        want_db = ctx.has_bias and ctx.needs_input_grad[2]
        if ctx.needs_input_grad[1] or want_db:
            co, ci = weight.shape[:2]
            if conv3x3_sb_wrw_wanted(x, dy):
                dw = _on_wgrad_stream(lambda: conv3x3_sb_wrw(x, dy, ax=ctx.ax, ady=ady), x, dy, ctx.ax, ady) \
                    if ctx.needs_input_grad[1] else None
                db = bias_grad(dy) if want_db else None
            elif not ctx.has_bias and co == ci and co in CONV3X3_WRW_CHANNELS and x.shape[3] % 4 == 0:
                dw = _conv3x3_wrw(x, dy, co, ci)
            else:
                _, dw, db = torch.ops.aten.convolution_backward(
                    dy, x, weight, [co] if ctx.has_bias else None, [1, 1], [1, 1], [1, 1], False, [0, 0], 1,
                    [False, bool(ctx.needs_input_grad[1]), bool(want_db)])
        return dx, dw, db, None


def conv3x3_split_bf16(x, weight, bias=None, want_stats=False):
    return Conv3x3SplitBF16.apply(x, weight, bias, want_stats)


class Conv3x3SplitFork(Function):

    @staticmethod
    def forward(ctx, x, weight, want_stats=False):
        weight = weight.contiguous()
        ctx.save_for_backward(x, weight)
        ctx.pick = weight.shape[0] in CONV3X3_SB_PICK_NT_CHANNELS
        ctx.ax = amax_of(x) if split_arith_id() else None
        nt = conv3x3_sb_pick_nt(x, weight.shape[0]) if ctx.pick else 0
        return conv3x3_sb_run(x, weight, False, None, nt, ax=ctx.ax, want_stats=want_stats), x.view_as(x)

    @staticmethod
    def backward(ctx, dy, g):
        x, weight = ctx.saved_tensors
        ady = amax_of(dy) if split_arith_id() else None
        dy = dy.contiguous()
        dx = None
        if ctx.needs_input_grad[0]:
            nt = conv3x3_sb_pick_nt(dy, weight.shape[1]) if ctx.pick else 0
            dx = conv3x3_sb_run(dy, weight, True, None, nt, ax=ady, addend=None if g is None else g.contiguous())
        dw = None
        if ctx.needs_input_grad[1]:
            co, ci = weight.shape[:2]
# ... 34 lines not shown
        out, mi2, am2 = _bn_train_fwd(c2, g2, b2, x, bn2)
        amax_attach(out, am2)
        ctx.save_for_backward(x, w1, g1, b1, w2, g2, b2, c1, a1, c2, out, mi1, mi2)
        ctx.misc = (nt, ax, am1)
        return out

    @staticmethod
    def backward(ctx, dy):
        x, w1, g1, b1, w2, g2, b2, c1, a1, c2, out, mi1, mi2 = ctx.saved_tensors
        nt, ax, am1 = ctx.misc
        dy = dy.contiguous()
        am = amax_request(c2)
        dc2, dg2, db2, g = bn_bwd(dy, c2, out, mi2, g2, b2, 2, True, True, amax=am)
        da1 = conv3x3_sb_run(dc2, w2, True, None, nt, ax=am)
        dw2 = _on_wgrad_stream(lambda: conv3x3_sb_wrw(a1, dc2, ax=am1, ady=am), a1, dc2, am1, am) if ctx.needs_input_grad[4] else None
        amb = amax_request(c1)
        dc1, dg1, db1, _ = bn_bwd(da1, c1, None, mi1, g1, b1, 1, True, True, amax=amb)
        dx = conv3x3_sb_run(dc1, w1, True, None, nt, ax=amb, addend=g) if ctx.needs_input_grad[0] else None
        dw1 = _on_wgrad_stream(lambda: conv3x3_sb_wrw(x, dc1, ax=ax, ady=amb), x, dc1, ax, amb) if ctx.needs_input_grad[1] else None
        return (dx, dw1, dg1 if g1 is not None else None, db1 if b1 is not None else None, dw2,
                dg2 if g2 is not None else None, db2 if b2 is not None else None, None, None, None, None)


def _bn_train_fwd(x, weight, bias, residual, bn):
    amax = amax_request(x)
    tiles = known_tile_stats(x)
    if tiles is not None:
        mi = bn_tiles_finalize(tiles, bn.eps, bn.momentum, bn.running_mean, bn.running_var, bn.num_batches_tracked)
        y = bn_apply(x, mi, weight, bias, residual, True, amax=amax)
    else:
        y, mi = bn_fwd(x, weight, bias, residual, True, bn.eps, bn.momentum, bn.running_mean, bn.running_var, bn.num_batches_tracked,
                       amax=amax)
    return y, mi, amax


def basic_block_split(x, blk):
    return BasicBlockSplit.apply(x, blk.conv1.weight, blk.bn1.weight, blk.bn1.bias, blk.conv2.weight, blk.bn2.weight, blk.bn2.bias,
                                 blk.bn1, blk.bn2, blk.conv1.bn_follows, blk.conv2.bn_follows)


BLOCK_GROUP = os.environ.get("CSEG_BLOCK_GROUP", "1") == "1"
NT_GROUP = _hip.NT_GROUP
_GROUP_SCHED = {}


def _group_sched(device):
    key = (device.index, _hip.raw_stream()) if device.type == "cuda" else (-1, 0)
    buf = _GROUP_SCHED.get(key)
    if buf is None:
        buf = _GROUP_SCHED[key] = torch.zeros(_hip.GROUP_SCHED_INTS, dtype=I32, device=device)
    return buf


def conv3x3_group_run(items, want_stats=False):
    n = len(items)
    arr = (_hip.ConvGroupMember * n)()
    ys, sts = [], []
    stats_on = want_stats and CONV_EPILOGUE_STATS
    for e, (x, weight, flip, ax, addend) in zip(arr, items):
        co, ci = weight.shape[:2]
        conv_in, conv_out = (co, ci) if flip else (ci, co)
        B, _, H, W = x.shape
        wp, aw = SPLIT_WEIGHTS.get(weight, "c3", flip, NT_GROUP)
        y = torch.empty(B, conv_out, H, W, dtype=F32, device=x.device)
        e.x, e.wp, e.y, e.amax_x, e.amax_w = _pq(x, "x").value, wp.data_ptr(), y.data_ptr(), ax.data_ptr(), aw.data_ptr()
        if addend is not None:
            e.addend = _pq(addend, "addend").value
        st = None
        if stats_on and addend is None:
            st = tile_stats_buffer(0, conv_out, B, H, W, x.device)
            e.stats = st.data_ptr()
            tile_stats_attach(y, st)
        e.B, e.Cin, e.Cout, e.H, e.W = B, conv_in, conv_out, H, W
        ys.append(y)
        sts.append(st)
    _hip.call("cseg_conv3x3_split_group_fwd", ctypes.byref(arr), n, split_arith_id(), _pf(_group_sched(ys[0].device)), _hip.stream_ptr())
    return ys, sts


def conv3x3_group_wrw(items):
    n = len(items)
    arr = (_hip.WrwGroupMember * n)()
    lib = _hip.lib()
    dws, keep = [], []
    for e, (x, dy, ax, ady) in zip(arr, items):
        B, ci, H, W = x.shape
        co = dy.shape[1]
        nf = lib.cseg_conv3x3_sb_wrw_ws_floats(B, ci, co, H, W)
        if nf == 0:
            raise RuntimeError("conv3x3_group_wrw: unsupported shape %s x %s" % (tuple(x.shape), tuple(dy.shape)))
        ws = torch.empty(nf, dtype=F32, device=x.device)
        dw = torch.empty(co, ci, 3, 3, dtype=F32, device=x.device)
        e.x, e.dy, e.amax_x, e.amax_dy, e.ws, e.dw = _pq(x, "x").value, _pq(dy, "dy").value, ax.data_ptr(), ady.data_ptr(), ws.data_ptr(), dw.data_ptr()
        e.B, e.Cin, e.Cout, e.H, e.W = B, ci, co, H, W
        dws.append(dw)
        keep.append(ws)
    _hip.call("cseg_conv3x3_split_group_wrw", ctypes.byref(arr), n, split_arith_id(), _hip.stream_ptr())
    return dws


def bn_group_fwd(xs, bns, residuals, relu):
    n = len(xs)
    arr = (_hip.BnGroupMember * n)()
    ys, mis, ams = [], [], []
    for e, x, bn, r in zip(arr, xs, bns, residuals):
        B, C, HW = _bn_dims(x)
        st = known_tile_stats(x)
        if st is None:
            raise RuntimeError("bn_group_fwd: an input without epilogue statistics")
        mi = torch.empty(C, 2, dtype=F32, device=x.device)
        y = torch.empty_like(x)
        am = amax_request(x)
        p, b = bn._parameters, bn._buffers
        e.x, e.y, e.stats, e.mean_invstd = x.data_ptr(), y.data_ptr(), st.data_ptr(), mi.data_ptr()
        if r is not None:
            e.residual = _pq(r, "residual").value
        w_, b_ = p.get("weight"), p.get("bias")
        if w_ is not None:
            e.weight = w_.data_ptr()
        if b_ is not None:
            e.bias = b_.data_ptr()
        rm, rv, nbt = b.get("running_mean"), b.get("running_var"), b.get("num_batches_tracked")
        if rm is not None:
            e.running_mean, e.running_var = rm.data_ptr(), rv.data_ptr()
        if nbt is not None:
            e.num_batches_tracked = nbt.data_ptr()
        if am is not None:
            e.amax_out = am.data_ptr()
        e.B, e.C, e.HW, e.T, e.eps, e.momentum = B, C, HW, st.shape[1], float(bn.eps), float(bn.momentum)
        ys.append(y)
        mis.append(mi)
        ams.append(am)
    sp = _hip.stream_ptr()
    _hip.call("cseg_bn_group_tiles_finalize", ctypes.byref(arr), n, sp)
    _hip.call("cseg_bn_group_apply", ctypes.byref(arr), n, int(bool(relu)), sp)
    return ys, mis, ams


_BN_GROUP_WS = {}


def bn_group_bwd(dys, xs, outs, mis, bns, mode):
    n = len(xs)
    arr = (_hip.BnGroupMember * n)()
    lib = _hip.lib()
    needs, total = [], 0
    for x in xs:
        B, C, HW = _bn_dims(x)
        nf = _BN_WS_NEED.get((B, C, HW))
        if nf is None:
            nf = _BN_WS_NEED[(B, C, HW)] = max(1, lib.cseg_bn_ws_floats(B, C, HW))
        needs.append(total)
        total += (nf + 63) // 64 * 64
    dev = xs[0].device
    key = (dev.index, _hip.raw_stream()) if dev.type == "cuda" else (-1, 0)
    ws = _BN_GROUP_WS.get(key)
    if ws is None or ws.numel() < total:
        ws = _BN_GROUP_WS[key] = torch.empty(max(total, 1 << 17), dtype=F32, device=dev)
    base = ws.data_ptr()
    res = []
    for e, dy, x, out, mi, bn, off in zip(arr, dys, xs, outs, mis, bns, needs):
        B, C, HW = _bn_dims(x)
        d_wb = torch.empty(2, C, dtype=F32, device=dev)
        g = torch.empty_like(x) if mode == 2 else None
        dx = torch.empty_like(x)
        am = amax_request(x)
        p = bn._parameters
        e.dy, e.x, e.mean_invstd, e.dx, e.ws = _pq(dy, "dy").value, x.data_ptr(), mi.data_ptr(), dx.data_ptr(), base + 4 * off
        e.d_weight, e.d_bias = d_wb.data_ptr(), d_wb.data_ptr() + 4 * C
        if mode == 2:
            e.out, e.g_masked = out.data_ptr(), g.data_ptr()
        w_, b_ = p.get("weight"), p.get("bias")
        if w_ is not None:
            e.weight = w_.data_ptr()
        if b_ is not None:
            e.bias = b_.data_ptr()
        if am is not None:
            e.amax_out = am.data_ptr()
        e.B, e.C, e.HW = B, C, HW
        res.append((dx, d_wb[0], d_wb[1], g, am))
# ... 333 lines not shown
            if ctx.needs_input_grad[1] else None
        db = bias_grad(dy) if (ctx.has_bias and ctx.needs_input_grad[2]) else None
        return dx, dw, db, None, None


def conv3x3_dilany_split(x, weight, bias, dil, want_stats=False):
    return Conv3x3DilAny.apply(x, weight, bias, dil, want_stats)


def conv3x3_split_fork(x, weight, want_stats=False):
    return Conv3x3SplitFork.apply(x, weight, want_stats)


CONV3X3_S2_SPLIT = os.environ.get("CSEG_CONV3X3_S2_SPLIT", "1") == "1"


def _s2_base_ok(x, weight):
    return (CONV3X3_S2_SPLIT and CONV3X3_SPLIT_BF16 and SPLIT_ARITH == "f16x3" and _on_device(x) and x.dtype == F32 and weight.dtype == F32 and x.dim() == 4
            and tuple(weight.shape[2:]) == (3, 3) and x.shape[2] % 2 == 0 and x.shape[3] % 2 == 0)


def conv3x3_s2_fwd_eligible(x, weight):
    co, ci = weight.shape[:2]
    return _s2_base_ok(x, weight) and x.shape[1] == ci and ci % 16 == 0 and (co % 48 == 0 or co % 64 == 0)


def conv3x3_s2_bwd_eligible(x, weight):
    co, ci = weight.shape[:2]
    return _s2_base_ok(x, weight) and co % 16 == 0 and (ci % 48 == 0 or ci % 64 == 0) and x.shape[3] % 4 == 0


def conv3x3_s2_wrw_eligible(x, weight):
    co, ci = weight.shape[:2]
    return _s2_base_ok(x, weight) and ci % 16 == 0 and co % 16 == 0 and x.shape[3] % 64 == 0


def conv3x3_s2_pick_nt(B, Ho, Wo, c_out):
    spatial = B * ((Ho + 3) // 4) * ((Wo + 63) // 64)
    if c_out % 48:
        return 4
    return 6 if c_out % 96 == 0 and spatial * (c_out // 96) >= 256 else 3


def conv3x3_s2_run(x, weight, ax=None, want_stats=False):
    co, ci = weight.shape[:2]
    B, _, H, W = x.shape
    Ho, Wo = H // 2, W // 2
    nt = conv3x3_s2_pick_nt(B, Ho, Wo, co)
    wp, aw = SPLIT_WEIGHTS.get(weight, "c3s2", False, nt)
    ax = tensor_amax(x) if ax is None else ax
    y = torch.empty(B, co, Ho, Wo, dtype=F32, device=x.device)
    if want_stats and CONV_EPILOGUE_STATS:
        st = tile_stats_buffer(0, co, B, Ho, Wo, x.device)
        _hip.call("cseg_conv3x3_s2_split_fwd_st", _p(x, F32, "x"), wp.data_ptr(), B, ci, co, Ho, Wo, nt, _pf(ax), _pf(aw), _pf(y),
                  _pf(st), _hip.stream_ptr())
        return tile_stats_attach(y, st)
    _hip.call("cseg_conv3x3_s2_split_fwd", _p(x, F32, "x"), wp.data_ptr(), B, ci, co, Ho, Wo, nt, _pf(ax), _pf(aw), _pf(y),
              _hip.stream_ptr())
    return y


def conv3x3_s2_bwd_run(dy, weight, ady=None):
    co, ci = weight.shape[:2]
    B, _, Ho, Wo = dy.shape
    nt = conv3x3_s2_pick_nt(B, Ho, Wo, ci)
    wp, aw = SPLIT_WEIGHTS.get(weight, "c3s2", True, nt)
    ady = tensor_amax(dy) if ady is None else ady
    dx = torch.empty(B, ci, 2 * Ho, 2 * Wo, dtype=F32, device=dy.device)
    _hip.call("cseg_conv3x3_s2_split_bwd", _p(dy, F32, "dy"), wp.data_ptr(), B, ci, co, Ho, Wo, nt, _pf(ady), _pf(aw), _pf(dx),
              _hip.stream_ptr())
    return dx


def conv3x3_s2_wrw(x, dy, ax=None, ady=None):
    B, ci, H, W = x.shape
    co, Ho, Wo = dy.shape[1:]
    n = _hip.lib().cseg_conv3x3_s2_wrw_ws_floats(B, ci, co, Ho, Wo)
    if n == 0 or (H, W) != (2 * Ho, 2 * Wo):
        raise RuntimeError("conv3x3_s2_wrw: unsupported shape %s x %s" % (tuple(x.shape), tuple(dy.shape)))
    ax = tensor_amax(x) if ax is None else ax
    ady = tensor_amax(dy) if ady is None else ady
    ws = torch.empty(n, dtype=F32, device=x.device)
    dw = torch.empty(co, ci, 3, 3, dtype=F32, device=x.device)
    _hip.call("cseg_conv3x3_s2_split_wrw", _p(x, F32, "x"), _p(dy, F32, "dy"), B, ci, co, Ho, Wo, split_arith_id(), _pf(ax), _pf(ady),
              _pf(ws), _pf(dw), _hip.stream_ptr())
    return dw


class Conv3x3S2Split(Function):

    @staticmethod
    def forward(ctx, x, weight, want_stats=False):
        weight = weight.contiguous()
        x = x.contiguous()
        ctx.save_for_backward(x, weight)
        ctx.ax = amax_of(x)
        if conv3x3_s2_fwd_eligible(x, weight):
            return conv3x3_s2_run(x, weight, ax=ctx.ax, want_stats=want_stats)
        return torch.nn.functional.conv2d(x, weight, None, 2, 1)

    @staticmethod
    def backward(ctx, dy):
        x, weight = ctx.saved_tensors
        co, ci = weight.shape[:2]
        ady = amax_of(dy)
        dy = dy.contiguous()
        need_dx, need_dw = bool(ctx.needs_input_grad[0]), bool(ctx.needs_input_grad[1])
        dx = dw = None
        if need_dx and conv3x3_s2_bwd_eligible(x, weight):
            dx = conv3x3_s2_bwd_run(dy, weight, ady=ady)
        if need_dw and conv3x3_s2_wrw_eligible(x, weight):
            dw = _on_wgrad_stream(lambda: conv3x3_s2_wrw(x, dy, ax=ctx.ax, ady=ady), x, dy, ctx.ax, ady)
        rest = [need_dx and dx is None, need_dw and dw is None, False]
        if rest[0] or rest[1]:
            gx, gw, _ = torch.ops.aten.convolution_backward(dy, x, weight, None, [2, 2], [1, 1], [1, 1], False, [0, 0], 1, rest)
            dx = gx if rest[0] else dx
            dw = gw if rest[1] else dw
        return dx, dw, None


def conv3x3_s2_split(x, weight, want_stats=False):
    return Conv3x3S2Split.apply(x, weight, want_stats)


CONV3X3_RGB_STEM = os.environ.get("CSEG_CONV3X3_RGB_STEM", "1") == "1"


def conv3x3_s2_rgb_eligible(x, weight):
    return (CONV3X3_RGB_STEM and _on_device(x) and x.dtype == F32 and weight.dtype == F32 and x.dim() == 4 and x.shape[1] == 3
            and tuple(weight.shape) == (64, 3, 3, 3) and x.shape[2] % 2 == 0 and x.shape[3] % 2 == 0 and not x.requires_grad)


class Conv3x3S2Rgb(Function):

    @staticmethod
    def forward(ctx, x, weight):
        x, weight = x.contiguous(), weight.contiguous()
        ctx.save_for_backward(x, weight)
        B, _, H, W = x.shape
        y = torch.empty(B, 64, H // 2, W // 2, dtype=F32, device=x.device)
        _hip.call("cseg_conv3x3_s2_rgb_fwd", _p(x, F32, "x"), _p(weight, F32, "weight"), B, 64, H, W, _pf(y), _hip.stream_ptr())
        return y

    @staticmethod
    def backward(ctx, dy):
        x, weight = ctx.saved_tensors
        if not ctx.needs_input_grad[1]:
            return None, None
        dy = dy.contiguous()
        B, _, H, W = x.shape
        n = _hip.lib().cseg_conv3x3_s2_rgb_wrw_ws_floats(B, 64, H, W)
        if n == 0:
            raise RuntimeError("conv3x3_s2_rgb_wrw: unsupported shape %s" % (tuple(x.shape),))

        def wrw():
            ws = torch.empty(n, dtype=F32, device=x.device)
            dw = torch.empty(64, 3, 3, 3, dtype=F32, device=x.device)
            _hip.call("cseg_conv3x3_s2_rgb_wrw", _p(x, F32, "x"), _p(dy, F32, "dy"), B, 64, H, W, _pf(ws), _pf(dw), _hip.stream_ptr())
            return dw
        return None, _on_wgrad_stream(wrw, x, dy)


def conv3x3_s2_rgb(x, weight):
    return Conv3x3S2Rgb.apply(x, weight)


CLS1X1 = os.environ.get("CSEG_CLS1X1", "1") == "1"
CLS1X1_MAX_K = 32
# ... 205 lines not shown
        if n == 0:
            raise RuntimeError("ocr_attn_bwd: unsupported shape %s x %s" % (tuple(q.shape), tuple(key.shape)))
        ws = torch.empty(n, dtype=F32, device=q.device)
        dq, dkey, dvalue = torch.empty_like(q), torch.empty_like(key), torch.empty_like(value)
        _hip.call("cseg_ocr_attn_bwd", _p(q, F32, "q"), _p(key, F32, "key"), _p(value, F32, "value"), _pf(stats), _p(dout, F32, "dout"),
                  ctx.scale, B, C, K_, KP, ctypes.c_long(P), _pf(ws), _pf(dq), _pf(dkey), _pf(dvalue), _hip.stream_ptr())
        return dq, dkey, dvalue, None, None


def ocr_attention(q, key, value, scale):
    return OcrAttention.apply(q, key, value, scale, torch.is_grad_enabled())


CONV1X1_SPLIT_BF16 = os.environ.get("CSEG_CONV1X1_SPLIT_BF16", "1") == "1"
CONV1X1_SB_MIN_TILES = int(os.environ.get("CSEG_SB_MIN_TILES", "1"))


def conv1x1_sb_eligible(x, weight):
    if not (_on_device(x) and x.dtype == F32 and weight.dtype == F32 and x.dim() == 4 and x.is_contiguous()):
        return False
    co, ci, kh, kw = weight.shape
    ok = lambda c: c % 48 == 0 or c % 64 == 0
    return (kh, kw) == (1, 1) and ok(ci) and ok(co) and x.shape[1] == ci


def conv1x1_sb_tiles(x, c_out):
    nt16 = next(16 * nt for nt in (9, 8, 6, 4, 3) if c_out % (16 * nt) == 0)
    return x.shape[0] * (c_out // nt16) * ((x.shape[2] * x.shape[3] + 255) // 256)


def conv1x1_sb_pack(weight, transpose=False):
    return SPLIT_WEIGHTS.get(weight, "c1", transpose, 0)


def conv1x1_sb_run(x, weight, transpose=False, bias=None, ax=None, want_stats=False, addend=None):
    co, ci = weight.shape[:2]
    conv_in, conv_out = (co, ci) if transpose else (ci, co)
    B, _, H, W = x.shape
    arith = split_arith_id()
    wp, aw = conv1x1_sb_pack(weight, transpose)
    if arith and ax is None:
        ax = tensor_amax(x)
    y = torch.empty(B, conv_out, H, W, dtype=F32, device=x.device)
    if want_stats and CONV_EPILOGUE_STATS:
        st = tile_stats_buffer(1, conv_out, B, H * W, 1, x.device)
        _hip.call("cseg_conv1x1_split_fwd_st", _pq(x, "x"), wp.data_ptr(), _opt(bias, F32, "bias"), B, conv_in, conv_out, H * W,
                  arith, _pf(ax) if arith else _null(), _pf(aw) if arith else _null(), _pf(y), _pf(st), _hip.stream_ptr())
        return tile_stats_attach(y, st)
    if addend is not None:
        _hip.call("cseg_conv1x1_split_fwd_add", _pq(x, "x"), wp.data_ptr(), _opt(bias, F32, "bias"), _pq(addend, "addend"), B, conv_in,
                  conv_out, H * W, arith, _pf(ax) if arith else _null(), _pf(aw) if arith else _null(), _pf(y), _hip.stream_ptr())
        return y
    _hip.call("cseg_conv1x1_split_fwd", _pq(x, "x"), wp.data_ptr(), _opt(bias, F32, "bias"), B, conv_in, conv_out, H * W,
              arith, _pf(ax) if arith else _null(), _pf(aw) if arith else _null(), _pf(y), _hip.stream_ptr())
    return y


CONV1X1_SB_WRW = os.environ.get("CSEG_CONV1X1_SB_WRW", "1") == "1"
CONV1X1_SB_WRW_MIN_CH = int(os.environ.get("CSEG_CONV1X1_SB_WRW_MIN_CH", "16"))


def conv1x1_sb_wrw_eligible(x, dy):
    return (_on_device(x) and x.dtype == F32 and dy.dtype == F32 and x.is_contiguous() and dy.is_contiguous()
            and x.shape[1] % 16 == 0 and dy.shape[1] % 16 == 0)


def conv1x1_sb_wrw_wanted(x, dy):
    return (CONV1X1_SB_WRW and min(x.shape[1], dy.shape[1]) >= CONV1X1_SB_WRW_MIN_CH and conv1x1_sb_wrw_eligible(x, dy))


def conv1x1_sb_wrw(x, dy, ax=None, ady=None):
    B, ci, H, W = x.shape
    co = dy.shape[1]
    lib = _hip.lib()
    n = lib.cseg_conv1x1_sb_wrw_ws_floats(B, ci, co, H * W)
    if n == 0:
        raise RuntimeError("conv1x1_sb_wrw: unsupported shape %s x %s" % (tuple(x.shape), tuple(dy.shape)))
    arith = split_arith_id()
    if arith:
        ax = tensor_amax(x) if ax is None else ax
        ady = tensor_amax(dy) if ady is None else ady
    ws = torch.empty(n, dtype=F32, device=x.device)
    dw = torch.empty(co, ci, 1, 1, dtype=F32, device=x.device)
    _hip.call("cseg_conv1x1_split_wrw", _pq(x, "x"), _pq(dy, "dy"), B, ci, co, H * W, arith,
              _pf(ax) if arith else _null(), _pf(ady) if arith else _null(), _pf(ws), _pf(dw), _hip.stream_ptr())
    return dw


class Conv1x1SplitBF16(Function):

    @staticmethod
    def forward(ctx, x, weight, bias, want_stats=False):
        weight = weight.contiguous()
        ctx.save_for_backward(x, weight)
        ctx.has_bias = bias is not None
        ctx.ax = amax_of(x) if split_arith_id() else None
        return conv1x1_sb_run(x, weight, False, bias, ax=ctx.ax, want_stats=want_stats)

    @staticmethod
    def backward(ctx, dy):
        x, weight = ctx.saved_tensors
        ady = amax_of(dy) if split_arith_id() else None
        dy = dy.contiguous()
        dx = conv1x1_sb_run(dy, weight, True, ax=ady) if ctx.needs_input_grad[0] else None
        dw = db = None
        want_db = ctx.has_bias and ctx.needs_input_grad[2]
        if conv1x1_sb_wrw_wanted(x, dy):
            dw = _on_wgrad_stream(lambda: conv1x1_sb_wrw(x, dy, ax=ctx.ax, ady=ady), x, dy, ctx.ax, ady) \
                if ctx.needs_input_grad[1] else None
            db = bias_grad(dy) if want_db else None
        elif ctx.needs_input_grad[1] or want_db:
            _, dw, db = torch.ops.aten.convolution_backward(
                dy, x, weight, [weight.shape[0]] if ctx.has_bias else None, [1, 1], [0, 0], [1, 1], False, [0, 0], 1,
                [False, bool(ctx.needs_input_grad[1]), bool(want_db)])
        return dx, dw, db, None


def conv1x1_split_bf16(x, weight, bias=None, want_stats=False):
    return Conv1x1SplitBF16.apply(x, weight, bias, want_stats)


class Conv1x1SplitSkip(Function):

    @staticmethod
    def forward(ctx, x, weight, bias, want_stats=False):
        weight = weight.contiguous()
        ctx.save_for_backward(x, weight)
        ctx.has_bias = bias is not None
        ctx.ax = amax_of(x) if split_arith_id() else None
        return conv1x1_sb_run(x, weight, False, bias, ax=ctx.ax, want_stats=want_stats), x.view_as(x)

    @staticmethod
    def backward(ctx, dy, dskip):
        x, weight = ctx.saved_tensors
        ady = amax_of(dy) if split_arith_id() else None
        dy = dy.contiguous()
        dx = None
        if ctx.needs_input_grad[0]:
            add = None
            if dskip is not None and dskip.dtype == F32 and dskip.shape == x.shape and _on_device(dskip):
                add = dskip.contiguous()
            dx = conv1x1_sb_run(dy, weight, True, ax=ady, addend=add)
            if dskip is not None and add is None:
                dx = dx + dskip
        dw = db = None
        want_db = ctx.has_bias and ctx.needs_input_grad[2]
        if conv1x1_sb_wrw_wanted(x, dy):
            dw = _on_wgrad_stream(lambda: conv1x1_sb_wrw(x, dy, ax=ctx.ax, ady=ady), x, dy, ctx.ax, ady) \
                if ctx.needs_input_grad[1] else None
            db = bias_grad(dy) if want_db else None
        elif ctx.needs_input_grad[1] or want_db:
            _, dw, db = torch.ops.aten.convolution_backward(
                dy, x, weight, [weight.shape[0]] if ctx.has_bias else None, [1, 1], [0, 0], [1, 1], False, [0, 0], 1,
                [False, bool(ctx.needs_input_grad[1]), bool(want_db)])
        return dx, dw, db, None


SKIP_ADD_FUSED = os.environ.get("CSEG_SKIP_ADD_FUSED", "1") == "1"


def conv1x1_split_skip(x, weight, bias=None, want_stats=False):
    y, skip = Conv1x1SplitSkip.apply(x, weight, bias, want_stats)
    a = getattr(x, "_cseg_amax", None)
    if a is not None and a[1] == x._version:
        skip._cseg_amax = (a[0], skip._version) + tuple(a[2:])
    return y, skip


# ... 46 lines not shown
```

### include/cseg_hip.h

```cpp
#ifndef CSEG_HIP_H
#define CSEG_HIP_H

#include <stddef.h>
#include <stdint.h>

#ifdef __cplusplus
extern "C" {
#endif

typedef void* cseg_stream_t;

int cseg_abi_version(void);
const char* cseg_last_error(void);

int cseg_classify_partition(const float* seg, const int64_t* pred_in, const int64_t* target, int B, int K, int h, int w, int H, int W,
                            int ignore_label, int32_t* lab, int32_t* pred, int16_t* key, int32_t* counts,
                            int32_t* seg_off, int32_t* part_idx, int32_t* status, cseg_stream_t stream);

int cseg_classify_partition_prezeroed(const float* seg, const int64_t* pred_in, const int64_t* target, int B, int K, int h, int w,
                                      int H, int W, int ignore_label, int32_t* lab, int32_t* pred, int16_t* key, int32_t* counts,
                                      int32_t* seg_off, int32_t* part_idx, int32_t* status, cseg_stream_t stream);

int cseg_gather_anchors(const float* embed, int B, int D, int P, const int32_t* part_idx,
                        const int32_t* sel_pos, int N, float* anchors, int32_t* sel_pix, cseg_stream_t stream);
// ... 162 lines not shown
int cseg_amax_f32(const float* x, long n, unsigned* amax_bits, cseg_stream_t stream);
#define CSEG_NT_SB8 0x109
size_t cseg_conv3x3_split_packed_bytes(int arith, int Cin, int Cout);
int cseg_conv3x3_split_pack(const float* w, int Cout, int Cin, int transpose_flip, int nt, int arith, const unsigned* amax_w,
                            void* wp, cseg_stream_t stream);
int cseg_conv3x3_split_fwd(const float* x, const void* wp, const float* bias, int B, int Cin, int Cout, int H, int W, int nt,
                           int arith, const unsigned* amax_x, const unsigned* amax_w, float* y, cseg_stream_t stream);
int cseg_conv3x3_split_fwd_add(const float* x, const void* wp, const float* bias, const float* addend, int B, int Cin, int Cout,
                               int H, int W, int nt, int arith, const unsigned* amax_x, const unsigned* amax_w, float* y,
                               cseg_stream_t stream);
int cseg_conv3x3_split_dil_fwd(const float* x, const void* wp, const float* bias, const float* addend, int B, int Cin, int Cout, int H,
                               int W, int dil, int arith, const unsigned* amax_x, const unsigned* amax_w, float* y, float* stats,
                               cseg_stream_t stream);
int cseg_conv3x3_split_dilany_plan(int conv_in, int conv_out, int* nt, long* threads);
size_t cseg_conv3x3_split_dilany_packed_bytes(int Cin, int Cout);
int cseg_conv3x3_split_dilany_pack(const float* w, int Cout, int Cin, int transpose_flip, const unsigned* amax_w, void* wp,
                                   cseg_stream_t stream);
int cseg_conv3x3_split_dilany_fwd(const float* x, const void* wp, const float* bias, const float* addend, int B, int Cin, int Cout,
                                  int H, int W, int dil, const unsigned* amax_x, const unsigned* amax_w, float* y, float* stats,
                                  cseg_stream_t stream);
size_t cseg_conv3x3_split_dilany_wrw_ws_floats(int B, int Cin, int Cout, int H, int W, int dil);
int cseg_conv3x3_split_dilany_wrw(const float* x, const float* dy, int B, int Cin, int Cout, int H, int W, int dil,
                                  const unsigned* amax_x, const unsigned* amax_dy, float* ws, float* dw, cseg_stream_t stream);
int cseg_conv3x3_split_wrw(const float* x, const float* dy, int B, int Cin, int Cout, int H, int W, int arith,
                           const unsigned* amax_x, const unsigned* amax_dy, float* ws, float* dw, cseg_stream_t stream);

#define CSEG_GROUP_MAX 8
#define CSEG_GROUP_SCHED_INTS 320
#define CSEG_NT_GROUP 0x203
typedef struct cseg_conv_group_member {
    const float* x;
    const void* wp;
    const float* bias;
    const float* addend;
    float* y;
    float* stats;
    const unsigned* amax_x;
    const unsigned* amax_w;
    int B, Cin, Cout, H, W;
    int reserved[3];
} cseg_conv_group_member;
int cseg_conv3x3_split_group_fwd(const cseg_conv_group_member* members, int n, int arith, int* sched, cseg_stream_t stream);
typedef struct cseg_bn_group_member {
    const float* x;
    const float* residual;
    float* y;
    const float* stats;
    float* mean_invstd;
    const float* weight;
    const float* bias;
    float* running_mean;
    float* running_var;
    int64_t* num_batches_tracked;
    unsigned* amax_out;
    const float* dy;
    const float* out;
    float* g_masked;
    float* d_weight;
    float* d_bias;
    float* dx;
    float* ws;
    int B, C, HW;
    long T;
    float eps, momentum;
} cseg_bn_group_member;
int cseg_bn_group_tiles_finalize(const cseg_bn_group_member* members, int n, cseg_stream_t stream);
int cseg_bn_group_apply(const cseg_bn_group_member* members, int n, int relu, cseg_stream_t stream);
int cseg_bn_group_bwd(const cseg_bn_group_member* members, int n, int mode, int training, cseg_stream_t stream);
int cseg_bn_group_tiles_moments(const cseg_bn_group_member* members, int n, double* packed, cseg_stream_t stream);
int cseg_bn_group_finalize(const cseg_bn_group_member* members, int n, const double* packed, cseg_stream_t stream);
int cseg_bn_group_bwd_reduce(const cseg_bn_group_member* members, int n, int mode, double* packed, cseg_stream_t stream);
int cseg_bn_group_bwd_apply(const cseg_bn_group_member* members, int n, int mode, const double* packed, cseg_stream_t stream);
typedef struct cseg_wrw_group_member {
    const float* x;
    const float* dy;
    const unsigned* amax_x;
    const unsigned* amax_dy;
    float* ws;
    float* dw;
    int B, Cin, Cout, H, W;
    int reserved[3];
} cseg_wrw_group_member;
int cseg_conv3x3_split_group_wrw(const cseg_wrw_group_member* members, int n, int arith, cseg_stream_t stream);
size_t cseg_conv3x3_s2_split_packed_bytes(int conv_in, int conv_out);
int cseg_conv3x3_s2_split_plan(int conv_in, int conv_out, int transposed, int nt, int* kind, long* threads);
int cseg_conv3x3_s2_split_pack(const float* w, int Cout, int Cin, int transposed, int nt, const unsigned* amax_w, void* wp,
                               cseg_stream_t stream);
int cseg_conv3x3_s2_split_fwd(const float* x, const void* wp, int B, int Cin, int Cout, int Ho, int Wo, int nt,
                              const unsigned* amax_x, const unsigned* amax_w, float* y, cseg_stream_t stream);
int cseg_conv3x3_s2_split_bwd(const float* dy, const void* wp, int B, int Cin, int Cout, int Ho, int Wo, int nt,
                              const unsigned* amax_dy, const unsigned* amax_w, float* dx, cseg_stream_t stream);
size_t cseg_conv3x3_s2_wrw_ws_floats(int B, int Cin, int Cout, int Ho, int Wo);
int cseg_conv3x3_s2_split_wrw(const float* x, const float* dy, int B, int Cin, int Cout, int Ho, int Wo, int arith,
                              const unsigned* amax_x, const unsigned* amax_dy, float* ws, float* dw, cseg_stream_t stream);
#define CSEG_PACK_C3 0
#define CSEG_PACK_C3_16 1
#define CSEG_PACK_C1 2
#define CSEG_PACK_C3_S2T 3
int cseg_conv3x3_split_plan(int conv_in, int conv_out, int nt_request, int* kind, int* nt, long* threads);
int cseg_conv1x1_split_plan(int conv_in, int conv_out, int* nt, long* threads);
int cseg_conv1x1_split_plan_arith(int arith, int conv_in, int conv_out, int* nt, long* threads);
typedef struct cseg_split_job {
    const void* src;
    void* dst;
    unsigned* amax;
    int cout, cin, flag, nt, kind, total, block0, reserved;
} cseg_split_job;
int cseg_amax_batch(const cseg_split_job* jobs_dev, int n_jobs, int total_blocks, cseg_stream_t stream);
int cseg_split_pack_batch(const cseg_split_job* jobs_dev, int n_jobs, int total_blocks, int arith, cseg_stream_t stream);
size_t cseg_conv1x1_split_packed_bytes(int arith, int Cin, int Cout);
int cseg_conv1x1_split_pack(const float* w, int Cout, int Cin, int transpose, int arith, const unsigned* amax_w, void* wp,
                            cseg_stream_t stream);
int cseg_conv1x1_split_fwd(const float* x, const void* wp, const float* bias, int B, int Cin, int Cout, int HW, int arith,
                           const unsigned* amax_x, const unsigned* amax_w, float* y, cseg_stream_t stream);
int cseg_conv1x1_split_fwd_add(const float* x, const void* wp, const float* bias, const float* addend, int B, int Cin, int Cout, int HW,
                               int arith, const unsigned* amax_x, const unsigned* amax_w, float* y, cseg_stream_t stream);
int cseg_conv1x1_split_wrw(const float* x, const float* dy, int B, int Cin, int Cout, int HW, int arith, const unsigned* amax_x,
                           const unsigned* amax_dy, float* ws, float* dw, cseg_stream_t stream);

int cseg_conv3x3_s2_rgb_fwd(const float* x, const float* w, int B, int Cout, int H, int W, float* y, cseg_stream_t stream);
size_t cseg_conv3x3_s2_rgb_wrw_ws_floats(int B, int Cout, int H, int W);
int cseg_conv3x3_s2_rgb_wrw(const float* x, const float* dy, int B, int Cout, int H, int W, float* ws, float* dw, cseg_stream_t stream);

int cseg_cls1x1_fwd(const float* x, const float* wt, const float* bias, int B, int C, int K, int KP, long P, float* y,
                    cseg_stream_t stream);
int cseg_cls1x1_bwd(const float* dy, const float* wt, int B, int C, int K, int KP, long P, float* dx, cseg_stream_t stream);
size_t cseg_cls1x1_wrw_ws_floats(int B, int C, int KP, long P);
int cseg_cls1x1_wrw(const float* x, const float* dy, int B, int C, int K, int KP, long P, float* ws, float* dwt, cseg_stream_t stream);

int cseg_cls1x1_wide_fwd(const float* x, const float* wt, const float* bias, int B, int C, int K, int KP, long P, float* y,
                         cseg_stream_t stream);
int cseg_cls1x1_wide_bwd(const float* dy, const float* wt, int B, int C, int K, int KP, long P, float* dx, cseg_stream_t stream);
size_t cseg_cls1x1_wide_wrw_ws_floats(int B, int C, int KP, long P);
int cseg_cls1x1_wide_wrw(const float* x, const float* dy, int B, int C, int K, int KP, long P, float* ws, float* dwt,
                         cseg_stream_t stream);

size_t cseg_ocr_gather_ws_floats(int B, int C, int K, int KP, long P);
int cseg_ocr_gather_fwd(const float* probs, const float* feats, float scale, int B, int C, int K, int KP, long P, float* ws,
                        float* rstats, float* ctx, cseg_stream_t stream);
int cseg_ocr_gather_bwd(const float* probs, const float* feats, const float* rstats, const float* dctx, float scale, int B, int C,
                        int K, int KP, long P, float* dprobs, float* dfeats, cseg_stream_t stream);
int cseg_ocr_attn_fwd(const float* q, const float* key, const float* value, float scale, int B, int C, int K, int KP, long P,
                      float* out, float* stats, cseg_stream_t stream);
size_t cseg_ocr_attn_bwd_ws_floats(int B, int C, int K, int KP, long P);
int cseg_ocr_attn_bwd(const float* q, const float* key, const float* value, const float* stats, const float* dout, float scale, int B,
                      int C, int K, int KP, long P, float* ws, float* dq, float* dkey, float* dvalue, cseg_stream_t stream);

#define CSEG_AUG_PARAM_INTS 12
int cseg_augment_batch(const uint8_t* img, const uint8_t* lab, const int16_t* lut, const int32_t* params, int B, int Hs,
                       int Ws, int Ht, int Wt, float div_value, const float* mean3, const float* std3, float* out_img,
                       int64_t* out_lab, cseg_stream_t stream);

int cseg_ms_fuse_argmax(int n_terms, const float* const* plain, const float* const* flipped, const int* hs, const int* ws,
                        const float* weights, int B, int K, int H, int W, uint8_t* pred, float* fused, cseg_stream_t stream);
int cseg_confusion_update(const uint8_t* pred, const int64_t* target, long N, int K, int ignore_index, int64_t* confusion,
                          cseg_stream_t stream);

int cseg_rmi_pool_blocks(int B, int K, int H, int W);
int cseg_rmi_pool_fwd(const float* seg, const int64_t* target, int B, int K, int h, int w, int H, int W, int rmi_radius,
                      int rmi_pool_way, int rmi_pool_size, int rmi_pool_stride, float* p_pool, uint8_t* route, uint8_t* l_pool,
                      double* partial, cseg_stream_t stream);
int cseg_rmi_cov(const float* p_pool, const uint8_t* l_pool, int B, int K, int hp, int wp, double* cov, double* means,
                 cseg_stream_t stream);
int cseg_rmi_solve(const double* cov, int n, double* rmi, double* grads, cseg_stream_t stream);
int cseg_rmi_finish(const double* partial, int n_blocks, const double* rmi, int B, int K, float lam, int lambda_way,
                    float loss_weight, double* outd, float* out, cseg_stream_t stream);
// ... 22 lines not shown
```

Before: 95.28 images/sec.

## Fuse split-K weight-gradient reduction into wrw kernels via last-arriver counters

Adds an arrive-counter path to the 3x3, grouped 3x3, strided 3x3 and 1x1 weight-gradient kernels. The last block to finish a tile sums the split partials and writes dw directly, so the separate reduce kernel launch is skipped; with a single split the kernel writes dw directly. By default the gate only enables this for the 1x1 family with n_split<=1, and an environment variable can widen it. This saves a kernel launch and a pass over the workspace, at the cost of atomics, fences and a serial tail in the last block.

```diff
diff --git a/contrastiveseg_amd/_hip.py b/contrastiveseg_amd/_hip.py
--- a/contrastiveseg_amd/_hip.py
+++ b/contrastiveseg_amd/_hip.py
@@ -40,6 +40,8 @@
 GROUP_MAX = 8
 GROUP_SCHED_INTS = 320
 NT_GROUP = 0x203
+WRW_ARRIVE_INTS = 4096
+WRW_3X3, WRW_3X3_GROUP, WRW_3X3_S2, WRW_1X1 = 0, 1, 2, 3
 
 
 SIGNATURES = {
@@ -104,6 +106,11 @@
     "cseg_conv3x3_split_fwd_add": (_c_int, [_ptr, _ptr, _ptr, _ptr] + [_c_int] * 7 + [_ptr, _ptr, _ptr, _ptr]),
     "cseg_conv3x3_split_group_fwd": (_c_int, [_ptr, _c_int, _c_int, _ptr, _ptr]),
     "cseg_conv3x3_split_group_wrw": (_c_int, [_ptr, _c_int, _c_int, _ptr]),
+    "cseg_wrw_combine_wanted": (_c_int, [_c_int] * 4),
+    "cseg_conv3x3_split_wrw_arrive": (_c_int, [_ptr, _ptr] + [_c_int] * 6 + [_ptr, _ptr, _ptr, _ptr, _ptr, _ptr]),
+    "cseg_conv3x3_split_group_wrw_arrive": (_c_int, [_ptr, _c_int, _c_int, _ptr, _ptr]),
+    "cseg_conv3x3_s2_split_wrw_arrive": (_c_int, [_ptr, _ptr] + [_c_int] * 6 + [_ptr, _ptr, _ptr, _ptr, _ptr, _ptr]),
+    "cseg_conv1x1_split_wrw_arrive": (_c_int, [_ptr, _ptr] + [_c_int] * 5 + [_ptr, _ptr, _ptr, _ptr, _ptr, _ptr]),
     "cseg_bn_group_tiles_finalize": (_c_int, [_ptr, _c_int, _ptr]),
     "cseg_bn_group_apply": (_c_int, [_ptr, _c_int, _c_int, _ptr]),
     "cseg_bn_group_bwd": (_c_int, [_ptr, _c_int, _c_int, _c_int, _ptr]),
diff --git a/contrastiveseg_amd/csrc/conv1x1_sb_wrw.hip b/contrastiveseg_amd/csrc/conv1x1_sb_wrw.hip
--- a/contrastiveseg_amd/csrc/conv1x1_sb_wrw.hip
+++ b/contrastiveseg_amd/csrc/conv1x1_sb_wrw.hip
@@ -16,7 +16,7 @@
                                                                 int B, int Cin, int Cout, int plane_i, int n_split,
                                                                 const unsigned* __restrict__ amax_x,
                                                                 const unsigned* __restrict__ amax_dy,
-                                                                float* __restrict__ partial) {
+                                                                float* __restrict__ partial, float* __restrict__ dw, int* arrive) {
     extern __shared__ __attribute__((aligned(16))) unsigned short smem_q[];
     constexpr int NP = AR::NP;
     constexpr int DY_ELEMS = dy_elems(NP), X_ELEMS = x_elems(NP);
@@ -182,6 +182,19 @@
             }
         }
     }
+    if (arrive) {
+        int* counter = arrive + cob * n_cib + cib;
+        if (!cseg_arrive_last(counter, n_split, reinterpret_cast<int*>(smem_q))) return;
+        const int co_n = min(CO_T, Cout - cob * CO_T), ci_n = min(CI_T, Cin - cib * CI_T);
+        const size_t total = (size_t)Cin * Cout;
+        for (int idx = tid; idx < co_n * CI_T; idx += 512) {
+            const int ci_l = idx % CI_T;
+            if (ci_l >= ci_n) continue;
+            const size_t e = (size_t)(cob * CO_T + idx / CI_T) * Cin + cib * CI_T + ci_l;
+            dw[e] = cseg_sum_splits(partial + e, total, n_split);
+        }
+        if (tid == 0) cseg_counter_store(counter, 0);
+    }
 }
 
 __global__ __launch_bounds__(256) void sb_wrw1_reduce_kernel(const float* __restrict__ partial, int n_split, int total,
@@ -231,7 +244,7 @@
 namespace {
 template <class AR, bool RAGGED>
 int launch_wrw1(const float* x, const float* dy, int B, int Cin, int Cout, int HW, int n_split, long blocks, const unsigned* amax_x,
-                const unsigned* amax_dy, float* ws, hipStream_t stream) {
+                const unsigned* amax_dy, float* ws, hipStream_t stream, float* dw = nullptr, int* arrive = nullptr) {
     const size_t lds = sizeof(unsigned short) * 2 * (dy_elems(AR::NP) + x_elems(AR::NP));
     static bool attr_set = false;
     if (!attr_set) {
@@ -243,13 +256,13 @@
         attr_set = true;
     }
     hipLaunchKernelGGL((conv1x1_sb_wrw_kernel<AR, RAGGED>), dim3((unsigned)blocks), dim3(512), lds, stream, x, dy, B, Cin, Cout, HW, n_split,
-                       amax_x, amax_dy, ws);
+                       amax_x, amax_dy, ws, dw, arrive);
     CSEG_CHECK_LAUNCH("conv1x1_sb_wrw_kernel");
     return 1;
 }
 
 int wrw1_impl(const float* x, const float* dy, int B, int Cin, int Cout, int HW, int arith, const unsigned* amax_x,
-              const unsigned* amax_dy, float* ws, float* dw, hipStream_t stream) {
+              const unsigned* amax_dy, float* ws, float* dw, hipStream_t stream, int* arrive = nullptr) {
     CSEG_REQUIRE(x && dy && ws && dw, "conv1x1_sb_wrw: null pointer");
     CSEG_REQUIRE(B > 0 && HW > 0 && Cin > 0 && Cout > 0 && Cin % 16 == 0 && Cout % 16 == 0,
                  "conv1x1_sb_wrw: unsupported shape B=%d Cin=%d Cout=%d HW=%d (needs channels %% 16)", B, Cin, Cout, HW);
@@ -263,14 +276,18 @@
     const int n_split = wrw1_splits(B, Cin, Cout, HW);
     const long blocks = (long)n_split * ((Cin + CI_T - 1) / CI_T) * ((Cout + CO_T - 1) / CO_T);
     CSEG_REQUIRE(blocks < 2147483647L && (long)Cin * Cout < 2147483647L, "conv1x1_sb_wrw: grid too large");
+    const bool combine = arrive && arith == CSEG_ARITH_F16X3 && cseg_wrw_combine_wanted(CSEG_WRW_FAMILY_1X1, n_split, Cin, Cout);
+    if (combine && n_split == 1) ws = dw;
+    if (!combine || n_split == 1) arrive = nullptr;
     int ok;
     if (arith == CSEG_ARITH_F16X3)
-        ok = ragged ? launch_wrw1<SplitF16x3, true>(x, dy, B, Cin, Cout, HW, n_split, blocks, amax_x, amax_dy, ws, stream)
-                    : launch_wrw1<SplitF16x3, false>(x, dy, B, Cin, Cout, HW, n_split, blocks, amax_x, amax_dy, ws, stream);
+        ok = ragged ? launch_wrw1<SplitF16x3, true>(x, dy, B, Cin, Cout, HW, n_split, blocks, amax_x, amax_dy, ws, stream, dw, arrive)
+                    : launch_wrw1<SplitF16x3, false>(x, dy, B, Cin, Cout, HW, n_split, blocks, amax_x, amax_dy, ws, stream, dw, arrive);
     else
         ok = ragged ? launch_wrw1<SplitBF16x6, true>(x, dy, B, Cin, Cout, HW, n_split, blocks, amax_x, amax_dy, ws, stream)
                     : launch_wrw1<SplitBF16x6, false>(x, dy, B, Cin, Cout, HW, n_split, blocks, amax_x, amax_dy, ws, stream);
     if (!ok) return 0;
+    if (combine) return 1;
     const int total = Cin * Cout;
     hipLaunchKernelGGL(sb_wrw1_reduce_kernel, dim3((total + 63) / 64), dim3(256), 0, stream, ws, n_split, total, dw);
     CSEG_CHECK_LAUNCH("sb_wrw1_reduce_kernel");
@@ -287,3 +304,8 @@
                                       const unsigned* amax_x, const unsigned* amax_dy, float* ws, float* dw, cseg_stream_t stream_) {
     return wrw1_impl(x, dy, B, Cin, Cout, HW, arith, amax_x, amax_dy, ws, dw, (hipStream_t)stream_);
 }
+extern "C" int cseg_conv1x1_split_wrw_arrive(const float* x, const float* dy, int B, int Cin, int Cout, int HW, int arith,
+                                             const unsigned* amax_x, const unsigned* amax_dy, float* ws, float* dw, int* arrive,
+                                             cseg_stream_t stream_) {
+    return wrw1_impl(x, dy, B, Cin, Cout, HW, arith, amax_x, amax_dy, ws, dw, (hipStream_t)stream_, arrive);
+}
diff --git a/contrastiveseg_amd/csrc/conv3x3_sb_wrw.hip b/contrastiveseg_amd/csrc/conv3x3_sb_wrw.hip
--- a/contrastiveseg_amd/csrc/conv3x3_sb_wrw.hip
+++ b/contrastiveseg_amd/csrc/conv3x3_sb_wrw.hip
@@ -212,12 +212,29 @@
 template <int NP, int SEGW>
 __device__ __forceinline__ int d2_idx(int buf, int p, int co, int i) { return ((buf * NP + p) * CO_B + co) * d2_pitch(NP, SEGW) + i; }
 
+__device__ __forceinline__ void sb_wrw_arrive_combine(const float* __restrict__ partial, int n_split, int Cout, int Cin, int cib, int cob,
+                                                      float* __restrict__ dw, int* counter, int* flag) {
+    if (!cseg_arrive_last(counter, n_split, flag)) return;
+    const int lane = threadIdx.x & 63, wave = threadIdx.x >> 6;
+    const int co_n = min(CO_B, Cout - cob * CO_B), ci = cib * CI_B + lane;
+    const size_t total = (size_t)9 * Cout * Cin;
+    if (ci < Cin) {
+        for (int row = wave; row < 9 * co_n; row += 8) {
+            const int tap = row / co_n, co = cob * CO_B + row - tap * co_n;
+            const size_t e = ((size_t)tap * Cout + co) * Cin + ci;
+            dw[((size_t)co * Cin + ci) * 9 + tap] = cseg_sum_splits(partial + e, total, n_split);
+        }
+    }
+    if (threadIdx.x == 0) cseg_counter_store(counter, 0);
+}
+
 template <class AR, int SEGW, int ABL = 0, bool RAGGED = false>
 __device__ __forceinline__ void conv3x3_sb_wrw2_body(const float* __restrict__ x, const float* __restrict__ dy,
                                                      int B, int Cin, int Cout, int H, int W, int n_split, int rpu,
                                                      int SC, int SI, const unsigned* __restrict__ amax_x,
                                                      const unsigned* __restrict__ amax_dy,
-                                                     float* __restrict__ partial, int bid, unsigned short* smem_w) {
+                                                     float* __restrict__ partial, int bid, unsigned short* smem_w,
+                                                     float* __restrict__ dw = nullptr, int* arrive = nullptr) {
     constexpr int NP = AR::NP;
     typedef typename AR::frag_t frag_t;
     unsigned short* xs = smem_w;
@@ -526,12 +543,20 @@
 #pragma unroll
                 for (int c = 0; c < 3; ++c) {
                     if (cob * CO_B + c * 16 >= Cout) continue;
+                    if (arrive && n_split == 1) {
+                        float* dst = dw + ((size_t)(cob * CO_B + c * 16 + 4 * g) * Cin + ci) * 9 + t;
+#pragma unroll
+                        for (int r = 0; r < 4; ++r) dst[(size_t)r * Cin * 9] = acc[t][c][r] * unscale;
+                        continue;
+                    }
                     float* dst = partial + (((size_t)split * 9 + t) * Cout + cob * CO_B + c * 16 + 4 * g) * Cin + ci;
 #pragma unroll
                     for (int r = 0; r < 4; ++r) dst[(size_t)r * Cin] = acc[t][c][r] * unscale;
                 }
         }
     }
+    if (arrive && n_split > 1)
+        sb_wrw_arrive_combine(partial, n_split, Cout, Cin, cib, cob, dw, arrive + cob * n_cib + cib, reinterpret_cast<int*>(smem_w));
 }
 
 template <class AR, int SEGW, int ABL = 0, bool RAGGED = false>
@@ -539,9 +564,10 @@
                                                                  int B, int Cin, int Cout, int H, int W, int n_split, int rpu,
                                                                  int SC, int SI, const unsigned* __restrict__ amax_x,
                                                                  const unsigned* __restrict__ amax_dy,
-                                                                 float* __restrict__ partial) {
+                                                                 float* __restrict__ partial, float* __restrict__ dw, int* arrive) {
     extern __shared__ __attribute__((aligned(16))) unsigned short smem_w2[];
-    conv3x3_sb_wrw2_body<AR, SEGW, ABL, RAGGED>(x, dy, B, Cin, Cout, H, W, n_split, rpu, SC, SI, amax_x, amax_dy, partial, (int)blockIdx.x, smem_w2);
+    conv3x3_sb_wrw2_body<AR, SEGW, ABL, RAGGED>(x, dy, B, Cin, Cout, H, W, n_split, rpu, SC, SI, amax_x, amax_dy, partial, (int)blockIdx.x, smem_w2,
+                                                dw, arrive);
 }
 
 __device__ __forceinline__ void sb_wrw_reduce_body(const float* __restrict__ partial, int n_split, int Cout, int Cin,
@@ -647,7 +673,7 @@
 
 template <class AR, int SEGW, int ABL = 0, bool RAGGED = false>
 int launch_wrw2(const float* x, const float* dy, int B, int Cin, int Cout, int H, int W, int n_split, const unsigned* amax_x,
-                const unsigned* amax_dy, float* ws, hipStream_t stream) {
+                const unsigned* amax_dy, float* ws, hipStream_t stream, float* dw = nullptr, int* arrive = nullptr) {
     const size_t lds2 = sizeof(unsigned short) * (x2_elems(AR::NP, SEGW) + d2_elems(AR::NP, SEGW));
     static bool attr2_set = false;
     if (!attr2_set) {
@@ -665,13 +691,13 @@
     const long blocks = ((n_groups + 7) / 8) * 8 * SC * SI;
     CSEG_REQUIRE(blocks < 2147483647L, "conv3x3_sb_wrw: grid too large");
     hipLaunchKernelGGL((conv3x3_sb_wrw2_kernel<AR, SEGW, ABL, RAGGED>), dim3((unsigned)blocks), dim3(512), lds2, stream, x, dy, B, Cin, Cout, H, W,
-                       n_split, wrw2_rpu(H), SC, SI, amax_x, amax_dy, ws);
+                       n_split, wrw2_rpu(H), SC, SI, amax_x, amax_dy, ws, dw, arrive);
     CSEG_CHECK_LAUNCH("conv3x3_sb_wrw2_kernel");
     return 1;
 }
 
 int wrw_impl(const float* x, const float* dy, int B, int Cin, int Cout, int H, int W, int arith, const unsigned* amax_x,
-             const unsigned* amax_dy, float* ws, float* dw, hipStream_t stream) {
+             const unsigned* amax_dy, float* ws, float* dw, hipStream_t stream, int* arrive = nullptr) {
     CSEG_REQUIRE(x && dy && ws && dw, "conv3x3_sb_wrw: null pointer");
     const bool v2 = arith == CSEG_ARITH_F16X3 || sb_wrw_version() == 2;
     const bool ragged = v2 && arith == CSEG_ARITH_F16X3 && wrw2_ragged(W);
@@ -682,8 +708,10 @@
     CSEG_REQUIRE(arith == CSEG_ARITH_BF16X6 || (arith == CSEG_ARITH_F16X3 && amax_x && amax_dy),
                  "conv3x3 split wrw: arithmetic %d needs max|x| and max|dy|", arith);
     const int n_split = sb_wrw_splits(B, Cin, Cout, H, W, arith);
-    const long blocks = (long)n_split * ((Cin + CI_B - 1) / CI_B) * ((Cout + CO_B - 1) / CO_B);
+    const long tiles = (long)((Cin + CI_B - 1) / CI_B) * ((Cout + CO_B - 1) / CO_B), blocks = (long)n_split * tiles;
     CSEG_REQUIRE(blocks < 2147483647L && (long)9 * Cin * Cout < 2147483647L, "conv3x3_sb_wrw: grid too large");
+    const bool combine = arrive && arith == CSEG_ARITH_F16X3 && cseg_wrw_combine_wanted(CSEG_WRW_FAMILY_3X3, n_split, Cin, Cout);
+    if (!combine) arrive = nullptr;
     if (v2) {
         CSEG_REQUIRE(ragged || ((reinterpret_cast<uintptr_t>(x) & 15) == 0 && (reinterpret_cast<uintptr_t>(dy) & 15) == 0),
                      "conv3x3_sb_wrw: tensors must be 16-byte aligned");
@@ -691,11 +719,11 @@
                      "conv3x3_sb_wrw: one image of x / dy must stay below 2 GiB (32-bit offsets)");
         const bool wide = wrw2_seg(W) == 64;
         const int ok = ragged
-                           ? (wide ? launch_wrw2<SplitF16x3, 64, 0, true>(x, dy, B, Cin, Cout, H, W, n_split, amax_x, amax_dy, ws, stream)
-                                   : launch_wrw2<SplitF16x3, 32, 0, true>(x, dy, B, Cin, Cout, H, W, n_split, amax_x, amax_dy, ws, stream))
+                           ? (wide ? launch_wrw2<SplitF16x3, 64, 0, true>(x, dy, B, Cin, Cout, H, W, n_split, amax_x, amax_dy, ws, stream, dw, arrive)
+                                   : launch_wrw2<SplitF16x3, 32, 0, true>(x, dy, B, Cin, Cout, H, W, n_split, amax_x, amax_dy, ws, stream, dw, arrive))
                        : arith == CSEG_ARITH_F16X3
-                           ? (wide ? launch_wrw2<SplitF16x3, 64>(x, dy, B, Cin, Cout, H, W, n_split, amax_x, amax_dy, ws, stream)
-                                   : launch_wrw2<SplitF16x3, 32>(x, dy, B, Cin, Cout, H, W, n_split, amax_x, amax_dy, ws, stream))
+                           ? (wide ? launch_wrw2<SplitF16x3, 64>(x, dy, B, Cin, Cout, H, W, n_split, amax_x, amax_dy, ws, stream, dw, arrive)
+                                   : launch_wrw2<SplitF16x3, 32>(x, dy, B, Cin, Cout, H, W, n_split, amax_x, amax_dy, ws, stream, dw, arrive))
                            : (wide ? launch_wrw2<SplitBF16x6, 64>(x, dy, B, Cin, Cout, H, W, n_split, amax_x, amax_dy, ws, stream)
                                    : launch_wrw2<SplitBF16x6, 32>(x, dy, B, Cin, Cout, H, W, n_split, amax_x, amax_dy, ws, stream));
         if (!ok) return 0;
@@ -714,6 +742,7 @@
                            n_split, ws);
         CSEG_CHECK_LAUNCH("conv3x3_sb_wrw_kernel");
     }
+    if (combine) return 1;
     const int total = 9 * Cin * Cout;
     hipLaunchKernelGGL(sb_wrw_reduce_kernel, dim3((total + 63) / 64), dim3(256), 0, stream, ws, n_split, Cout, Cin, dw);
     CSEG_CHECK_LAUNCH("sb_wrw_reduce_kernel");
@@ -723,6 +752,7 @@
 
 struct WrwGM {
     const float* x; const float* dy; const unsigned* amax_x; const unsigned* amax_dy; float* ws; float* dw;
+    int* arrive;
     int B, Cin, Cout, H, W, n_split, rpu, SC, SI, kind, block0, rblock0;
 };
 struct WrwGArgs { WrwGM m[CSEG_GROUP_MAX]; int n; };
@@ -734,7 +764,7 @@
     for (int i = 1; i < a.n; ++i) mi = (int)blockIdx.x >= a.m[i].block0 ? i : mi;
     const WrwGM& M = a.m[mi];
     conv3x3_sb_wrw2_body<SplitF16x3, SEGW, 0, false>(M.x, M.dy, M.B, M.Cin, M.Cout, M.H, M.W, M.n_split, M.rpu, M.SC, M.SI, M.amax_x, M.amax_dy, M.ws,
-                                                     (int)blockIdx.x - M.block0, smem_wg);
+                                                     (int)blockIdx.x - M.block0, smem_wg, M.dw, M.arrive);
 }
 __global__ __launch_bounds__(256) void sb_wrw_reduce_group_kernel(const WrwGArgs a) {
     int mi = 0;
@@ -759,7 +789,7 @@
     return 1;
 }
 
-int wrw_group_impl(const cseg_wrw_group_member* mem, int n, hipStream_t stream) {
+int wrw_group_impl(const cseg_wrw_group_member* mem, int n, hipStream_t stream, int* arrive = nullptr) {
     bool any_ragged = false;
     for (int i = 0; i < n; ++i) {
         const cseg_wrw_group_member& s = mem[i];
@@ -772,12 +802,12 @@
     if (any_ragged) {
         for (int i = 0; i < n; ++i)
             if (!wrw_impl(mem[i].x, mem[i].dy, mem[i].B, mem[i].Cin, mem[i].Cout, mem[i].H, mem[i].W, CSEG_ARITH_F16X3, mem[i].amax_x, mem[i].amax_dy,
-                          mem[i].ws, mem[i].dw, stream))
+                          mem[i].ws, mem[i].dw, stream, arrive))
                 return 0;
         return 1;
     }
     WrwGArgs all;
-    long rblocks = 0;
+    long rblocks = 0, tiles = 0;
     for (int i = 0; i < n; ++i) {
         const cseg_wrw_group_member& s = mem[i];
         CSEG_REQUIRE((reinterpret_cast<uintptr_t>(s.x) & 15) == 0 && (reinterpret_cast<uintptr_t>(s.dy) & 15) == 0,
@@ -793,8 +823,21 @@
         sb_wrw_group(n_cob, n_cib, m.SC, m.SI);
         m.kind = wrw2_seg(s.W) == 64 ? 0 : 1;
         m.block0 = 0;
-        m.rblock0 = (int)rblocks;
-        rblocks += (9L * s.Cin * s.Cout + 63) / 64;
+        const long mt = (long)n_cob * n_cib;
+        m.arrive = nullptr;
+        m.rblock0 = 0;
+        if (arrive && tiles + mt <= CSEG_WRW_ARRIVE_INTS && cseg_wrw_combine_wanted(CSEG_WRW_FAMILY_3X3_GROUP, m.n_split, s.Cin, s.Cout)) {
+            m.arrive = arrive + tiles;
+            tiles += mt;
+        }
+    }
+    WrwGArgs red;
+    int nr = 0;
+    for (int i = 0; i < n; ++i) {
+        if (all.m[i].arrive) continue;
+        red.m[nr] = all.m[i];
+        red.m[nr++].rblock0 = (int)rblocks;
+        rblocks += (9L * all.m[i].Cin * all.m[i].Cout + 63) / 64;
         CSEG_REQUIRE(rblocks < 2147483647L, "conv3x3 group wrw: grid too large");
     }
     for (int i = n; i < CSEG_GROUP_MAX; ++i) all.m[i] = all.m[0];
@@ -818,7 +861,10 @@
         a.n = k;
         if (!(kind == 0 ? launch_wrw2_group<64>(a, blocks, stream) : launch_wrw2_group<32>(a, blocks, stream))) return 0;
     }
-    hipLaunchKernelGGL(sb_wrw_reduce_group_kernel, dim3((unsigned)rblocks), dim3(256), 0, stream, all);
+    if (nr == 0) return 1;
+    for (int i = nr; i < CSEG_GROUP_MAX; ++i) red.m[i] = red.m[0];
+    red.n = nr;
+    hipLaunchKernelGGL(sb_wrw_reduce_group_kernel, dim3((unsigned)rblocks), dim3(256), 0, stream, red);
     CSEG_CHECK_LAUNCH("sb_wrw_reduce_group_kernel");
     return 1;
 }
@@ -829,6 +875,11 @@
     CSEG_REQUIRE(mem && n >= 1 && n <= CSEG_GROUP_MAX, "conv3x3 group wrw: needs 1 .. %d members", CSEG_GROUP_MAX);
     CSEG_REQUIRE(arith == CSEG_ARITH_F16X3, "conv3x3 group wrw: f16x3 arithmetic only (got %d)", arith);
     return wrw_group_impl(mem, n, (hipStream_t)stream_);
+}
+extern "C" int cseg_conv3x3_split_group_wrw_arrive(const cseg_wrw_group_member* mem, int n, int arith, int* arrive, cseg_stream_t stream_) {
+    CSEG_REQUIRE(mem && n >= 1 && n <= CSEG_GROUP_MAX, "conv3x3 group wrw: needs 1 .. %d members", CSEG_GROUP_MAX);
+    CSEG_REQUIRE(arith == CSEG_ARITH_F16X3, "conv3x3 group wrw: f16x3 arithmetic only (got %d)", arith);
+    return wrw_group_impl(mem, n, (hipStream_t)stream_, arrive);
 }
 
 namespace {
@@ -847,7 +898,7 @@
                                                                    int B, int Cin, int Cout, int Ho, int Wo, int n_split, int rpu,
                                                                    int SC, int SI, const unsigned* __restrict__ amax_x,
                                                                    const unsigned* __restrict__ amax_dy,
-                                                                   float* __restrict__ partial) {
+                                                                   float* __restrict__ partial, float* __restrict__ dw, int* arrive) {
     extern __shared__ __attribute__((aligned(16))) unsigned short smem_w[];
     constexpr int NP = AR::NP;
     typedef typename AR::frag_t frag_t;
@@ -1081,12 +1132,20 @@
 #pragma unroll
                 for (int c = 0; c < 3; ++c) {
                     if (cob * CO_B + c * 16 >= Cout) continue;
+                    if (arrive && n_split == 1) {
+                        float* dst = dw + ((size_t)(cob * CO_B + c * 16 + 4 * g) * Cin + ci) * 9 + t;
+#pragma unroll
+                        for (int r = 0; r < 4; ++r) dst[(size_t)r * Cin * 9] = acc[t][c][r] * unscale;
+                        continue;
+                    }
                     float* dst = partial + (((size_t)split * 9 + t) * Cout + cob * CO_B + c * 16 + 4 * g) * Cin + ci;
 #pragma unroll
                     for (int r = 0; r < 4; ++r) dst[(size_t)r * Cin] = acc[t][c][r] * unscale;
                 }
         }
     }
+    if (arrive && n_split > 1)
+        sb_wrw_arrive_combine(partial, n_split, Cout, Cin, cib, cob, dw, arrive + cob * n_cib + cib, reinterpret_cast<int*>(smem_w));
 }
 
 void s2_plan(int B, int Cin, int Cout, int Ho, int Wo, int& rpu, int& n_split) {
@@ -1119,10 +1178,9 @@
     return (size_t)n_split * 9 * Cin * Cout;
 }
 
-extern "C" int cseg_conv3x3_s2_split_wrw(const float* x, const float* dy, int B, int Cin, int Cout, int Ho, int Wo, int arith,
-                                         const unsigned* amax_x, const unsigned* amax_dy, float* ws, float* dw,
-                                         cseg_stream_t stream_) {
-    hipStream_t stream = (hipStream_t)stream_;
+namespace {
+int s2_wrw_impl(const float* x, const float* dy, int B, int Cin, int Cout, int Ho, int Wo, int arith, const unsigned* amax_x,
+                const unsigned* amax_dy, float* ws, float* dw, hipStream_t stream, int* arrive) {
     CSEG_REQUIRE(x && dy && ws && dw, "conv3x3_s2_wrw: null pointer");
     CSEG_REQUIRE(s2_shape_ok(B, Cin, Cout, Ho, Wo), "conv3x3_s2_wrw: unsupported shape B=%d Cin=%d Cout=%d out %dx%d (needs Cin %% 16, Cout %% 16, Wo %% 32)",
                  B, Cin, Cout, Ho, Wo);
@@ -1150,14 +1208,28 @@
     const long n_groups = (long)n_split * (n_cob / SC) * (n_cib / SI);
     const long blocks = ((n_groups + 7) / 8) * 8 * SC * SI;
     CSEG_REQUIRE(blocks < 2147483647L, "conv3x3_s2_wrw: grid too large");
+    if (!(arrive && cseg_wrw_combine_wanted(CSEG_WRW_FAMILY_3X3_S2, n_split, Cin, Cout))) arrive = nullptr;
     hipLaunchKernelGGL((conv3x3_sb_wrw_s2_kernel<SplitF16x3>), dim3((unsigned)blocks), dim3(512), lds, stream, x, dy, B, Cin, Cout, Ho, Wo,
-                       n_split, rpu, SC, SI, amax_x, amax_dy, ws);
+                       n_split, rpu, SC, SI, amax_x, amax_dy, ws, dw, arrive);
     CSEG_CHECK_LAUNCH("conv3x3_sb_wrw_s2_kernel");
+    if (arrive) return 1;
     const int total = 9 * Cin * Cout;
     hipLaunchKernelGGL(sb_wrw_reduce_kernel, dim3((total + 63) / 64), dim3(256), 0, stream, ws, n_split, Cout, Cin, dw);
     CSEG_CHECK_LAUNCH("sb_wrw_reduce_kernel");
     return 1;
 }
+}
+
+extern "C" int cseg_conv3x3_s2_split_wrw(const float* x, const float* dy, int B, int Cin, int Cout, int Ho, int Wo, int arith,
+                                         const unsigned* amax_x, const unsigned* amax_dy, float* ws, float* dw,
+                                         cseg_stream_t stream_) {
+    return s2_wrw_impl(x, dy, B, Cin, Cout, Ho, Wo, arith, amax_x, amax_dy, ws, dw, (hipStream_t)stream_, nullptr);
+}
+extern "C" int cseg_conv3x3_s2_split_wrw_arrive(const float* x, const float* dy, int B, int Cin, int Cout, int Ho, int Wo, int arith,
+                                                const unsigned* amax_x, const unsigned* amax_dy, float* ws, float* dw, int* arrive,
+                                                cseg_stream_t stream_) {
+    return s2_wrw_impl(x, dy, B, Cin, Cout, Ho, Wo, arith, amax_x, amax_dy, ws, dw, (hipStream_t)stream_, arrive);
+}
 
 extern "C" int cseg_conv3x3_sb_wrw(const float* x, const float* dy, int B, int Cin, int Cout, int H, int W, float* ws,
                                    float* dw, cseg_stream_t stream_) {
@@ -1169,3 +1241,19 @@
                                       cseg_stream_t stream_) {
     return wrw_impl(x, dy, B, Cin, Cout, H, W, arith, amax_x, amax_dy, ws, dw, (hipStream_t)stream_);
 }
+extern "C" int cseg_conv3x3_split_wrw_arrive(const float* x, const float* dy, int B, int Cin, int Cout, int H, int W, int arith,
+                                             const unsigned* amax_x, const unsigned* amax_dy, float* ws, float* dw, int* arrive,
+                                             cseg_stream_t stream_) {
+    return wrw_impl(x, dy, B, Cin, Cout, H, W, arith, amax_x, amax_dy, ws, dw, (hipStream_t)stream_, arrive);
+}
+
+extern "C" int cseg_wrw_combine_wanted(int family, int n_split, int Cin, int Cout) {
+    if (family < 0 || family > CSEG_WRW_FAMILY_1X1 || n_split < 1 || Cin < 1 || Cout < 1) return 0;
+    const bool one = family == CSEG_WRW_FAMILY_1X1;
+    const long tiles = (long)((Cin + (one ? 128 : CI_B) - 1) / (one ? 128 : CI_B)) * ((Cout + (one ? 144 : CO_B) - 1) / (one ? 144 : CO_B));
+    if (tiles > CSEG_WRW_ARRIVE_INTS) return 0;
+    const char* e = getenv("CSEG_WRW_COMBINE");
+    if (e && *e) return atoi(e) != 0;
+    static const int split_limit[4] = {0, 0, 0, 1};
+    return n_split <= split_limit[family];
+}
diff --git a/contrastiveseg_amd/csrc/cseg_common.h b/contrastiveseg_amd/csrc/cseg_common.h
--- a/contrastiveseg_amd/csrc/cseg_common.h
+++ b/contrastiveseg_amd/csrc/cseg_common.h
@@ -58,6 +58,52 @@
 #else
     __atomic_store_n(p, v, __ATOMIC_SEQ_CST);
 #endif
+}
+__device__ __forceinline__ void cseg_stores_drain() {
+#if defined(__AMDGCN__)
+    asm volatile("s_waitcnt vmcnt(0)" ::: "memory");
+#endif
+}
+__device__ __forceinline__ bool cseg_arrive_last(int* counter, int n, int* flag) {
+    cseg_stores_drain();
+    __syncthreads();
+    if (threadIdx.x == 0) {
+        cseg_release_agent();
+        const int last = cseg_counter_add(counter, 1) == n - 1;
+        if (last) {
+            cseg_acquire_agent();
+            cseg_stores_drain();
+        }
+        *flag = last;
+    }
+    __syncthreads();
+    return *flag != 0;
+}
+__device__ __forceinline__ float cseg_sum_splits(const float* __restrict__ p, size_t stride, int n_split) {
+    float s[4][4], r[4];
+#pragma unroll
+    for (int w = 0; w < 4; ++w)
+#pragma unroll
+        for (int k = 0; k < 4; ++k) s[w][k] = 0.f;
+    int base = 0;
+    for (; base + 16 <= n_split; base += 16)
+#pragma unroll
+        for (int w = 0; w < 4; ++w)
+#pragma unroll
+            for (int k = 0; k < 4; ++k) s[w][k] += p[(size_t)(base + w + 4 * k) * stride];
+#pragma unroll
+    for (int w = 0; w < 4; ++w) {
+        int sp = base + w;
+        for (; sp + 12 < n_split; sp += 16) {
+            s[w][0] += p[(size_t)sp * stride];
+            s[w][1] += p[(size_t)(sp + 4) * stride];
+            s[w][2] += p[(size_t)(sp + 8) * stride];
+            s[w][3] += p[(size_t)(sp + 12) * stride];
+        }
+        for (; sp < n_split; sp += 4) s[w][0] += p[(size_t)sp * stride];
+        r[w] = (s[w][0] + s[w][1]) + (s[w][2] + s[w][3]);
+    }
+    return (r[0] + r[1]) + (r[2] + r[3]);
 }
 #ifndef CSEG_SPIN_PAUSE
 #if defined(__AMDGCN__)
diff --git a/contrastiveseg_amd/kernels.py b/contrastiveseg_amd/kernels.py
--- a/contrastiveseg_amd/kernels.py
+++ b/contrastiveseg_amd/kernels.py
@@ -1460,6 +1460,23 @@
     return CONV3X3_SB_WRW and (same or (x.shape[1], dy.shape[1]) in CONV3X3_SB_WRW_PAIRS) and conv3x3_sb_wrw_eligible(x, dy)
 
 
+_WRW_ARRIVE = {}
+
+
+def _wrw_arrive(device):
+    key = (device.index, _hip.raw_stream()) if device.type == "cuda" else (-1, 0)
+    buf = _WRW_ARRIVE.get(key)
+    if buf is None:
+        buf = _WRW_ARRIVE[key] = torch.zeros(_hip.WRW_ARRIVE_INTS, dtype=I32, device=device)
+    return buf
+
+
+def _wrw_entry(name, family, ws_floats, taps, ci, co, device):
+    if _hip.lib().cseg_wrw_combine_wanted(family, ws_floats // (taps * ci * co), ci, co):
+        return name + "_arrive", (_pf(_wrw_arrive(device)),)
+    return name, ()
+
+
 def conv3x3_sb_wrw(x, dy, ax=None, ady=None):
     B, ci, H, W = x.shape
     co = dy.shape[1]
@@ -1473,8 +1490,9 @@
         ady = tensor_amax(dy) if ady is None else ady
     ws = torch.empty(n, dtype=F32, device=x.device)
     dw = torch.empty(co, ci, 3, 3, dtype=F32, device=x.device)
-    _hip.call("cseg_conv3x3_split_wrw", _pq(x, "x"), _pq(dy, "dy"), B, ci, co, H, W, arith,
-              _pf(ax) if arith else _null(), _pf(ady) if arith else _null(), _pf(ws), _pf(dw), _hip.stream_ptr())
+    entry, arrive = _wrw_entry("cseg_conv3x3_split_wrw", _hip.WRW_3X3, n, 9, ci, co, x.device) if arith else ("cseg_conv3x3_split_wrw", ())
+    _hip.call(entry, _pq(x, "x"), _pq(dy, "dy"), B, ci, co, H, W, arith,
+              _pf(ax) if arith else _null(), _pf(ady) if arith else _null(), _pf(ws), _pf(dw), *arrive, _hip.stream_ptr())
     return dw
 
 
@@ -1675,7 +1693,7 @@
     n = len(items)
     arr = (_hip.WrwGroupMember * n)()
     lib = _hip.lib()
-    dws, keep = [], []
+    dws, keep, wanted = [], [], False
     for e, (x, dy, ax, ady) in zip(arr, items):
         B, ci, H, W = x.shape
         co = dy.shape[1]
@@ -1688,7 +1706,11 @@
         e.B, e.Cin, e.Cout, e.H, e.W = B, ci, co, H, W
         dws.append(dw)
         keep.append(ws)
-    _hip.call("cseg_conv3x3_split_group_wrw", ctypes.byref(arr), n, split_arith_id(), _hip.stream_ptr())
+        wanted = wanted or bool(lib.cseg_wrw_combine_wanted(_hip.WRW_3X3_GROUP, nf // (9 * ci * co), ci, co))
+    if wanted:
+        _hip.call("cseg_conv3x3_split_group_wrw_arrive", ctypes.byref(arr), n, split_arith_id(), _pf(_wrw_arrive(dws[0].device)), _hip.stream_ptr())
+    else:
+        _hip.call("cseg_conv3x3_split_group_wrw", ctypes.byref(arr), n, split_arith_id(), _hip.stream_ptr())
     return dws
 
 
@@ -2188,8 +2210,9 @@
     ady = tensor_amax(dy) if ady is None else ady
     ws = torch.empty(n, dtype=F32, device=x.device)
     dw = torch.empty(co, ci, 3, 3, dtype=F32, device=x.device)
-    _hip.call("cseg_conv3x3_s2_split_wrw", _p(x, F32, "x"), _p(dy, F32, "dy"), B, ci, co, Ho, Wo, split_arith_id(), _pf(ax), _pf(ady),
-              _pf(ws), _pf(dw), _hip.stream_ptr())
+    entry, arrive = _wrw_entry("cseg_conv3x3_s2_split_wrw", _hip.WRW_3X3_S2, n, 9, ci, co, x.device)
+    _hip.call(entry, _p(x, F32, "x"), _p(dy, F32, "dy"), B, ci, co, Ho, Wo, split_arith_id(), _pf(ax), _pf(ady),
+              _pf(ws), _pf(dw), *arrive, _hip.stream_ptr())
     return dw
 
 
@@ -2561,8 +2584,9 @@
         ady = tensor_amax(dy) if ady is None else ady
     ws = torch.empty(n, dtype=F32, device=x.device)
     dw = torch.empty(co, ci, 1, 1, dtype=F32, device=x.device)
-    _hip.call("cseg_conv1x1_split_wrw", _pq(x, "x"), _pq(dy, "dy"), B, ci, co, H * W, arith,
-              _pf(ax) if arith else _null(), _pf(ady) if arith else _null(), _pf(ws), _pf(dw), _hip.stream_ptr())
+    entry, arrive = _wrw_entry("cseg_conv1x1_split_wrw", _hip.WRW_1X1, n, 1, ci, co, x.device) if arith else ("cseg_conv1x1_split_wrw", ())
+    _hip.call(entry, _pq(x, "x"), _pq(dy, "dy"), B, ci, co, H * W, arith,
+              _pf(ax) if arith else _null(), _pf(ady) if arith else _null(), _pf(ws), _pf(dw), *arrive, _hip.stream_ptr())
     return dw
 
 
diff --git a/include/cseg_hip.h b/include/cseg_hip.h
--- a/include/cseg_hip.h
+++ b/include/cseg_hip.h
@@ -268,6 +268,20 @@
     int reserved[3];
 } cseg_wrw_group_member;
 int cseg_conv3x3_split_group_wrw(const cseg_wrw_group_member* members, int n, int arith, cseg_stream_t stream);
+#define CSEG_WRW_ARRIVE_INTS 4096
+#define CSEG_WRW_FAMILY_3X3 0
+#define CSEG_WRW_FAMILY_3X3_GROUP 1
+#define CSEG_WRW_FAMILY_3X3_S2 2
+#define CSEG_WRW_FAMILY_1X1 3
+int cseg_wrw_combine_wanted(int family, int n_split, int Cin, int Cout);
+int cseg_conv3x3_split_wrw_arrive(const float* x, const float* dy, int B, int Cin, int Cout, int H, int W, int arith,
+                                  const unsigned* amax_x, const unsigned* amax_dy, float* ws, float* dw, int* arrive, cseg_stream_t stream);
+int cseg_conv3x3_split_group_wrw_arrive(const cseg_wrw_group_member* members, int n, int arith, int* arrive, cseg_stream_t stream);
+int cseg_conv3x3_s2_split_wrw_arrive(const float* x, const float* dy, int B, int Cin, int Cout, int Ho, int Wo, int arith,
+                                     const unsigned* amax_x, const unsigned* amax_dy, float* ws, float* dw, int* arrive,
+                                     cseg_stream_t stream);
+int cseg_conv1x1_split_wrw_arrive(const float* x, const float* dy, int B, int Cin, int Cout, int HW, int arith, const unsigned* amax_x,
+                                  const unsigned* amax_dy, float* ws, float* dw, int* arrive, cseg_stream_t stream);
 size_t cseg_conv3x3_s2_split_packed_bytes(int conv_in, int conv_out);
 int cseg_conv3x3_s2_split_plan(int conv_in, int conv_out, int transposed, int nt, int* kind, long* threads);
 int cseg_conv3x3_s2_split_pack(const float* w, int Cout, int Cin, int transposed, int nt, const unsigned* amax_w, void* wp,
```

Result: no change. 95.81 images/sec, median of 4 (+0.6%).
